# thimabru1010/ResUnet-a_mltsk_keras

Measured on AMD Instinct MI355X. Metric: training patches/sec (256×256, 6-ch, bs=8/GPU) at 1/2/4/8 MI355X, higher is better.
Workload: dtype bf16; 1 GPU; cfg3: ResUnet-a d6 multitask (seg+bound+dist+color) Tanimoto-dual, 256x256x6, 6 classes, Adam, full train step (fwd+loss+bwd+allreduce+update); global_batch=8, per_gpu_batch=8, parallelism=dp1

## Files before the change

include/rua_hip.h:

```cpp
#ifndef RUA_HIP_H
#define RUA_HIP_H
#include <stdint.h>
#ifdef __cplusplus
extern "C" {
#endif

#define RUA_F32 0
#define RUA_BF16 1
#define RUA_MAX_SEG 6
#define RUA_MAX_BRANCH 4
#define RUA_MAX_WGRAD_BATCH 32
#define RUA_MAX_WGRAD_GROUP 8

#define RUA_OK 0
#define RUA_ERR_ARG (-1)
#define RUA_ERR_LAUNCH (-2)

int rua_version(void);
const char* rua_last_error(void);
int rua_device_info(int* cu_count, int* lds_bytes, char* arch, int arch_len);

typedef struct rua_conv_seg {
  const void* x;
  const void* w;
  int32_t C, Hs, Ws;
  int32_t up_shift;
  int32_t dil;
  int32_t taps;
} rua_conv_seg;

typedef struct rua_bn_fold {
  const double* stats;
  int32_t replicas, pad;
  double count, bessel_n;
  float eps, momentum;
  const float* gamma; const float* beta;
  float* moving_mean; float* moving_var;
  float* scale; float* shift; float* mean; float* rstd;
} rua_bn_fold;

typedef struct rua_conv_desc {
  rua_conv_seg seg[RUA_MAX_SEG];
  int32_t nseg;
  int32_t N, H, W, Cout;
  int32_t stride;
  int32_t dtype;
  const float* bias;
  const void* aux;
  int32_t aux_mode;
  const float* mscale;
  const float* mshift;
  int32_t out_relu;
  int32_t accumulate;
  void* y;
  int32_t out_stride, OH, OW;
  double* stats;
  int32_t stats_mode;
  void* workspace;
  int64_t workspace_bytes;
  int32_t stats_replicas;
  const float* bias_more[3];
  const float* in_scale;
  const float* in_shift;
  int32_t in_relu;
  int32_t pad_fold;
  const struct rua_bn_fold* in_fold;
} rua_conv_desc;
int rua_conv_fwd(const rua_conv_desc* d, void* stream);
int rua_conv_fwd_group(const rua_conv_desc* d, int n, void* stream);
int rua_conv_group_last_grids(void);
int rua_conv_group_band_ok(const rua_conv_desc* d, int n);
int rua_conv_group_last_band(void);
int rua_conv_group_last_chain(void);
int rua_conv_fwd_sum(const rua_conv_desc* d, int n, void* stream);
int rua_conv_sum_last_kernel(void);
int rua_conv_sum_kernel(const rua_conv_desc* d, int n);
int rua_conv_smem_bytes(const rua_conv_desc* d);
int64_t rua_conv_workspace_bytes(const rua_conv_desc* d);
void* rua_prof_event_create(void);
int rua_prof_event_record(void* ev, void* hip_stream);
int rua_prof_event_elapsed_us(void* start, void* stop, double* us);
void rua_prof_event_destroy(void* ev);
void rua_profile_mid_event(void* hip_event);
int rua_profile_mid_event_fired(void);
int rua_conv_last_ksplit(void);
int rua_conv_tile_bn(const rua_conv_desc* d);
int rua_conv_kernel_id(const rua_conv_desc* d);
int rua_conv_fused_input_ok(const rua_conv_desc* d);
int rua_conv_tile_bm(const rua_conv_desc* d);

typedef struct rua_wgrad_desc {
  const void* a;  int32_t C, Hs, Ws;
  const void* dy; int32_t Cout, H, W;
  int32_t N, stride, dil, taps, dtype;
  float* dw;
  void* workspace;
  int64_t workspace_bytes;
  const float* in_scale;
  const float* in_shift;
  int32_t in_relu;
  int32_t defer;
  int32_t group_members;
  int32_t batch;
  const int32_t* overwrite_dev;
} rua_wgrad_desc;
typedef struct rua_wgrad_pending {
  int32_t kind;
  int32_t parts;
  int64_t n;
  const float* partials;
  float* dw;
  int32_t CC;
  int32_t blocks;
  int32_t block_begin, pad;
  const int32_t* overwrite_dev;
} rua_wgrad_pending;
int rua_wgrad_plan(const rua_wgrad_desc* d, rua_wgrad_pending* out);
int rua_wgrad_reduce_batch(const rua_wgrad_pending* items_dev, int n_items, int total_blocks, void* stream);
int rua_conv_wgrad(const rua_wgrad_desc* d, void* stream);
int rua_conv_wgrad_group(const rua_wgrad_desc* d, int n, void* stream);
int rua_wgrad_group_last_grids(void);
int rua_wgrad_group_plan(const rua_wgrad_desc* d, int n, rua_wgrad_pending* out);
int64_t rua_wgrad_workspace_bytes(const rua_wgrad_desc* d);
int rua_wgrad_kind(const rua_wgrad_desc* d);
int rua_wgrad_img_kind(const rua_wgrad_desc* d);

typedef struct rua_wprep_item { int64_t src_off, dst_off; int32_t taps, Cout, C, pad; } rua_wprep_item;
int rua_weight_prep(const float* master, void* w_fwd, void* w_dgrad, const rua_wprep_item* items_dev,
                    int n_items, int max_elems, int dtype, void* stream);
int rua_weight_prep_dgrad(const void* w_fwd, void* w_dgrad, const rua_wprep_item* items_dev, int n_items, int max_elems, const int32_t* blockmap_dev,
                          int n_blocks, int dtype, void* stream);
int rua_wprep_blocks(int taps, int Cout, int C);

int rua_stem_fwd(const float* x, const float* w, const float* b, void* y, int64_t M, int Cin, int Cout, int dtype, void* stream);
int rua_stem_fwd_stats(const float* x, const float* w, const float* b, void* y, int64_t M, int Cin, int Cout, int dtype, double* stats, int replicas, void* stream);
int rua_stem_bwd(const float* x, const void* dy, float* dw, float* db, int64_t M, int Cin, int Cout, int dtype, void* stream);
int rua_stem_fwd_pack(const float* x, const float* w, const float* b, void* y, int64_t M, int Cin, int Cout, int dtype, double* stats, int replicas,
                      void* xpack, void* stream);
int rua_stem_bwd_fold(float* tmp, float* dw, float* db, int Cin, int Cout, void* stream);
int rua_head_fwd(const void* x, const float* w, const float* b, float* z, float* p, int64_t M, int Cin, int Cout, int act, int dtype, void* stream);
int rua_head_fwd_loss(const void* x, const float* w, const float* b, float* z, float* p, const float* y, double* tanimoto_sums,
                      double* metrics, int B, int64_t HW, int Cin, int Cout, int act, int dtype, void* stream);
int rua_head_fwd_loss_rep(const void* x, const float* w, const float* b, float* z, float* p, const float* y, double* tanimoto_sums,
                          int sums_replicas, double* metrics, int B, int64_t HW, int Cin, int Cout, int act, int dtype, void* stream);
int rua_head_bwd(const void* x, const float* dz, const float* w, void* dx, int accumulate_dx, float* dw, float* db,
                 float* scratch, int64_t scratch_bytes, int64_t M, int Cin, int Cout, int dtype, int mask_dx, void* stream);
int rua_head_bwd_sums(const void* x, const float* dz, const float* w, void* dx, int accumulate_dx, float* dw, float* db, float* dxsum,
                      float* scratch, int64_t scratch_bytes, int64_t M, int Cin, int Cout, int dtype, int mask_dx, void* stream);

int rua_col_stats(const void* x, int64_t M, int C, double* stats, int replicas, int dtype, void* stream);
int rua_stats_replicas(int64_t blocks);
int rua_col_stats2(const void* g, const void* x, const float* mscale, const float* mshift, int masked,
                   int64_t M, int C, double* stats, int replicas, int dtype, void* stream);
int rua_bn_finalize(const double* stats, int replicas, double count, double bessel_n, const float* gamma, const float* beta,
                    float* moving_mean, float* moving_var, float momentum, float eps, int training,
                    float* scale, float* shift, float* mean, float* rstd, int C, void* stream);
int rua_stats_to_f32(const double* stats, int replicas, int C, float* const* dst, int n, void* stream);
int rua_bn_apply(const void* x, int nb, const float* const* scale, const float* const* shift, int relu,
                 void* const* out, int64_t M, int C, int dtype, void* stream);
int rua_bn_bwd_finalize(const double* stats2, int replicas, double count, const float* gamma, const float* mean, const float* rstd,
                        float* dgamma, float* dbeta, float* coefA, float* coefB, float* coefC, int C, void* stream);
int rua_bn_bwd_apply(int nb, const void* const* g, const float* const* coefA, const float* const* coefB,
                     const float* const* coefC, const float* const* mscale, const float* const* mshift, int masked,
                     const void* x, const void* dskip, void* dx, int accumulate, int64_t M, int C, int dtype, void* stream);

typedef struct rua_bn_branch {
  const float* gamma; const float* beta; float* moving_mean; float* moving_var;
  float* scale; float* shift; float* mean; float* rstd;
  void* out;
  const double* stats; int32_t replicas, pad;
  double* out_stats;
} rua_bn_branch;
typedef struct rua_bn_fwd_desc {
  const void* x; int64_t M; int32_t C, dtype, nb, relu, training, replicas;
  const double* stats;
  double count, bessel_n; float momentum, eps;
  rua_bn_branch br[RUA_MAX_BRANCH];
} rua_bn_fwd_desc;
int rua_bn_fwd(const rua_bn_fwd_desc* d, void* stream);
int rua_bn_fwd_group(const rua_bn_fwd_desc* d, int n, void* stream);
int rua_bn_fwd_group_last_grids(void);
typedef struct rua_bn_bwd_branch {
  const void* g; const double* stats2; int32_t replicas;
  int32_t stats2_out;
  const float* gamma; const float* mean; const float* rstd; const float* scale; const float* shift;
  float* dgamma; float* dbeta;
} rua_bn_bwd_branch;
typedef struct rua_bn_bwd_desc {
  const void* x; const void* dskip; void* dx; int64_t M; int32_t C, dtype, nb, masked, accumulate, pad; double count;
  rua_bn_bwd_branch br[RUA_MAX_BRANCH];
  double* skip_stats;
  int32_t skip_replicas, pad2;
  double* dx_stats;
  int32_t dx_replicas, pad3;
} rua_bn_bwd_desc;
int rua_bn_bwd(const rua_bn_bwd_desc* d, void* stream);
int rua_bn_bwd_group(const rua_bn_bwd_desc* d, int n, void* stream);
int rua_bn_bwd_group_last_grids(void);

int rua_maxpool_fwd(const void* x, void* y, uint8_t* idx, int N, int H, int W, int C, int k, int dtype, void* stream);
int rua_maxpool_bwd(const void* dy, const uint8_t* idx, void* dx, int accumulate, int N, int H, int W, int C, int k, int dtype, void* stream);
int rua_sumpool(const void* x, void* y, int N, int H, int W, int C, int k, int dtype, void* stream);
int rua_maxpool_derive(const void* y_half, const uint8_t* idx_half, void* y, uint8_t* idx, int N, int H_half, int W_half, int C,
                       int k_half, int dtype, void* stream);
int rua_maxpool_bwd_multi(int n, const void* const* dy, const uint8_t* const* idx, const int* ks, void* dx, int accumulate,
                          int N, int H, int W, int C, int dtype, void* stream);
int rua_sumpool_pyramid(const void* x, void* y2, void* y4, void* y8, int N, int H, int W, int C, int dtype, void* stream);
int rua_upsample_nearest(const void* x, void* y, int N, int H, int W, int C, int k, int dtype, void* stream);

int rua_add_n(int n, const void* const* in, void* out, int accumulate, int64_t elems, int dtype, void* stream);
int rua_relu_mask(void* dy, const void* y, int64_t elems, int dtype, void* stream);
int rua_relu(const void* x, void* y, int64_t elems, int dtype, void* stream);
int rua_cast_f32_to(const float* x, void* y, int64_t elems, int dtype, void* stream);
int rua_cast_to_f32(const void* x, float* y, int64_t elems, int dtype, void* stream);
int rua_fill_zero(void* p, int64_t bytes, void* stream);

#define RUA_LOSS_TANIMOTO 0
#define RUA_LOSS_WCE 1
#define RUA_LOSS_CE_LOGITS 2
#define RUA_LOSS_BCE_LOGITS 3
#define RUA_LOSS_MSE 4
#define RUA_ACT_NONE 0
#define RUA_ACT_SOFTMAX 1
#define RUA_ACT_SIGMOID 2
int rua_tanimoto_sums(const float* p, const float* y, int B, int64_t HW, int C, double* sums, void* stream);
int rua_tanimoto_finalize(const double* sums, int B, int64_t HW, int C, float grad_scale, double* loss_out, float* coef,
                          float* per_sample, void* stream);
#define RUA_MAX_HEADS 8
typedef struct rua_tani_head {
  double* sums; int32_t replicas, B, C; float grad_scale; double* loss_out; float* coef; float* per_sample;
} rua_tani_head;
int rua_tanimoto_finalize_multi(const rua_tani_head* heads, int n, void* stream);
typedef struct rua_dz_head {
  int32_t kind, act; const float* p; const float* y; const float* coef; const float* class_w; float grad_scale; int32_t B; int64_t HW; int32_t C, pad; float* dz;
} rua_dz_head;
int rua_head_dz_multi(const rua_dz_head* heads, int n, void* stream);
int rua_tanimoto_finalize_rep(double* sums, int replicas, int B, int64_t HW, int C, float grad_scale, double* loss_out, float* coef,
                              float* per_sample, void* stream);
int rua_tanimoto_ratio(const double* sums, int B, int C, double* mean_out, float* per_sample, void* stream);
int rua_pixel_loss(int kind, const float* p, const float* z, const float* y, const float* class_w,
                   int64_t M, int C, double* loss_out, float* per_pixel, void* stream);
int rua_head_dz(int kind, int act, const float* p, const float* y, const float* coef, const float* class_w,
                float grad_scale, int B, int64_t HW, int C, float* dz, void* stream);
int rua_seg_metrics(const float* p, const float* y, int64_t M, int C, double* out, void* stream);

int rua_tanimoto_sums_void(const float* p, const float* y, const uint8_t* void_mask, int B, int64_t HW, int C, double* sums, void* stream);
int rua_head_fwd_loss_void(const void* x, const float* w, const float* b, float* z, float* p, const float* y, double* tanimoto_sums,
                           int sums_replicas, double* metrics, int B, int64_t HW, int Cin, int Cout, int act, int dtype,
                           const uint8_t* void_mask, void* stream);
int rua_pixel_loss_void(int kind, const float* p, const float* z, const float* y, const float* class_w, const uint8_t* void_mask,
                        int64_t M, int C, double* loss_out, float* per_pixel, void* stream);
int rua_head_dz_void(int kind, int act, const float* p, const float* y, const float* coef, const float* class_w,
                     float grad_scale, int B, int64_t HW, int C, const uint8_t* void_mask, float* dz, void* stream);
int rua_head_dz_multi_void(const rua_dz_head* heads, int n, const uint8_t* void_mask, void* stream);
int rua_seg_metrics_void(const float* p, const float* y, const uint8_t* void_mask, int64_t M, int C, double* out, void* stream);

int rua_lr_step(double* state, float* lr_out, int adam, double beta1, double beta2, void* stream);
int rua_adam_step(float* theta, float* g, float* m, float* v, int64_t n, float lr_t, const float* lr_t_dev, float beta1, float beta2,
                  float eps, float grad_scale, int zero_grad, void* stream);
int rua_sgd_step(float* theta, float* g, float* vel, int64_t n, float lr, const float* lr_dev, float momentum, float grad_scale,
                 int zero_grad, void* stream);
int rua_adam_step_w(float* theta, float* g, float* m, float* v, int64_t n, float lr_t, const float* lr_t_dev, float beta1, float beta2,
                    float eps, float grad_scale, int zero_grad, void* wcopy_bf16, void* stream);
int rua_sgd_step_w(float* theta, float* g, float* vel, int64_t n, float lr, const float* lr_dev, float momentum, float grad_scale,
                   int zero_grad, void* wcopy_bf16, void* stream);

int64_t rua_targets_scratch_bytes(int N, int num_classes);
int rua_multitask_targets(const uint8_t* img, const uint8_t* cls, int N, int H, int W, int Cin, int num_classes, int norm_type,
                          float* x, float* seg, float* bound, float* dist, float* color, void* scratch, int64_t scratch_bytes, void* stream);
int rua_void_mask(const uint8_t* cls, int N, int H, int W, int num_classes, int margin, uint8_t* mask, void* stream);

int rua_scene_windows(const uint8_t* const* scene_img, const uint8_t* const* scene_cls, const int32_t* scene_h, const int32_t* scene_w,
                      int nscenes, const int32_t* windows, int N, int PH, int PW, int Cin,
                      uint8_t* img_out, uint8_t* cls_out, void* stream);

int rua_scene_windows_affine(const uint8_t* const* scene_img, const uint8_t* const* scene_cls, const int32_t* scene_h, const int32_t* scene_w,
                             int nscenes, const int32_t* windows , int N, int PH, int PW, int Cin,
// ... 36 lines not shown
```

resunet_a_mltsk_keras_amd/_lib.py:

```python
from __future__ import annotations

import ctypes as C
import os

HERE = os.path.dirname(os.path.abspath(__file__))
LIB_PATH = os.environ.get("RUA_LIB_PATH") or os.path.join(HERE, "librua_hip.so")

RUA_F32, RUA_BF16 = 0, 1
RUA_MAX_SEG, RUA_MAX_BRANCH, RUA_MAX_WGRAD_GROUP, RUA_MAX_WGRAD_BATCH = 6, 4, 8, 32
LOSS_TANIMOTO, LOSS_WCE, LOSS_CE_LOGITS, LOSS_BCE_LOGITS, LOSS_MSE = 0, 1, 2, 3, 4
ACT_NONE, ACT_SOFTMAX, ACT_SIGMOID = 0, 1, 2

vp, i32, i64, f32, f64 = C.c_void_p, C.c_int32, C.c_int64, C.c_float, C.c_double


class ConvSeg(C.Structure):
    _fields_ = [("x", vp), ("w", vp), ("C", i32), ("Hs", i32), ("Ws", i32), ("up_shift", i32), ("dil", i32), ("taps", i32)]


class ConvDesc(C.Structure):
    _fields_ = [("seg", ConvSeg * RUA_MAX_SEG), ("nseg", i32), ("N", i32), ("H", i32), ("W", i32), ("Cout", i32),
                ("stride", i32), ("dtype", i32), ("bias", vp), ("aux", vp), ("aux_mode", i32), ("mscale", vp),
                ("mshift", vp), ("out_relu", i32), ("accumulate", i32), ("y", vp), ("out_stride", i32), ("OH", i32),
                ("OW", i32), ("stats", vp), ("stats_mode", i32), ("workspace", vp), ("workspace_bytes", i64), ("stats_replicas", i32),
                ("bias_more", vp * 3), ("in_scale", vp), ("in_shift", vp), ("in_relu", i32), ("pad_fold", i32), ("in_fold", vp)]


class BnFold(C.Structure):
    _fields_ = [("stats", vp), ("replicas", i32), ("pad", i32), ("count", f64), ("bessel_n", f64), ("eps", f32), ("momentum", f32),
                ("gamma", vp), ("beta", vp), ("moving_mean", vp), ("moving_var", vp), ("scale", vp), ("shift", vp), ("mean", vp), ("rstd", vp)]


class WgradDesc(C.Structure):
    _fields_ = [("a", vp), ("C", i32), ("Hs", i32), ("Ws", i32), ("dy", vp), ("Cout", i32), ("H", i32), ("W", i32),
                ("N", i32), ("stride", i32), ("dil", i32), ("taps", i32), ("dtype", i32), ("dw", vp), ("workspace", vp), ("workspace_bytes", i64),
                ("in_scale", vp), ("in_shift", vp), ("in_relu", i32), ("defer", i32), ("group_members", i32), ("batch", i32), ("overwrite_dev", vp)]


class WgradPending(C.Structure):
    _fields_ = [("kind", i32), ("parts", i32), ("n", i64), ("partials", vp), ("dw", vp), ("CC", i32), ("blocks", i32),
                ("block_begin", i32), ("pad", i32), ("overwrite_dev", vp)]


class TaniHead(C.Structure):
    _fields_ = [("sums", vp), ("replicas", i32), ("B", i32), ("C", i32), ("grad_scale", f32), ("loss_out", vp), ("coef", vp), ("per_sample", vp)]


class DzHead(C.Structure):
    _fields_ = [("kind", i32), ("act", i32), ("p", vp), ("y", vp), ("coef", vp), ("class_w", vp), ("grad_scale", f32), ("B", i32), ("HW", i64),
                ("C", i32), ("pad", i32), ("dz", vp)]


class BnBranch(C.Structure):
    _fields_ = [("gamma", vp), ("beta", vp), ("moving_mean", vp), ("moving_var", vp), ("scale", vp), ("shift", vp),
                ("mean", vp), ("rstd", vp), ("out", vp), ("stats", vp), ("replicas", i32), ("pad", i32), ("out_stats", vp)]


class BnFwdDesc(C.Structure):
    _fields_ = [("x", vp), ("M", i64), ("C", i32), ("dtype", i32), ("nb", i32), ("relu", i32), ("training", i32), ("replicas", i32),
                ("stats", vp), ("count", f64), ("bessel_n", f64), ("momentum", f32), ("eps", f32), ("br", BnBranch * RUA_MAX_BRANCH)]


class BnBwdBranch(C.Structure):
    _fields_ = [("g", vp), ("stats2", vp), ("replicas", i32), ("stats2_out", i32), ("gamma", vp), ("mean", vp), ("rstd", vp),
                ("scale", vp), ("shift", vp), ("dgamma", vp), ("dbeta", vp)]


class BnBwdDesc(C.Structure):
    _fields_ = [("x", vp), ("dskip", vp), ("dx", vp), ("M", i64), ("C", i32), ("dtype", i32), ("nb", i32), ("masked", i32),
                ("accumulate", i32), ("pad", i32), ("count", f64), ("br", BnBwdBranch * RUA_MAX_BRANCH),
                ("skip_stats", vp), ("skip_replicas", i32), ("pad2", i32), ("dx_stats", vp), ("dx_replicas", i32), ("pad3", i32)]


class WprepItem(C.Structure):
    _fields_ = [("src_off", i64), ("dst_off", i64), ("taps", i32), ("Cout", i32), ("C", i32), ("pad", i32)]


PP = C.POINTER(vp)

_SIGS = {
    "rua_version": ([], i32),
    "rua_device_info": ([C.POINTER(i32), C.POINTER(i32), C.c_char_p, i32], i32),
    "rua_conv_fwd": ([C.POINTER(ConvDesc), vp], i32),
    "rua_conv_fwd_group": ([C.POINTER(ConvDesc), i32, vp], i32),
    "rua_conv_smem_bytes": ([C.POINTER(ConvDesc)], i32),
    "rua_conv_tile_bn": ([C.POINTER(ConvDesc)], i32),
    "rua_conv_tile_bm": ([C.POINTER(ConvDesc)], i32),
    "rua_conv_kernel_id": ([C.POINTER(ConvDesc)], i32),
    "rua_conv_fused_input_ok": ([C.POINTER(ConvDesc)], i32),
    "rua_conv_last_ksplit": ([], i32),
    "rua_conv_group_last_grids": ([], i32),
    "rua_conv_group_band_ok": ([C.POINTER(ConvDesc), i32], i32),
    "rua_conv_group_last_band": ([], i32),
    "rua_conv_group_last_chain": ([], i32),
    "rua_conv_fwd_sum": ([C.POINTER(ConvDesc), i32, vp], i32),
    "rua_conv_sum_last_kernel": ([], i32),
    "rua_conv_sum_kernel": ([C.POINTER(ConvDesc), i32], i32),
    "rua_conv_wgrad_group": ([C.POINTER(WgradDesc), i32, vp], i32),
    "rua_wgrad_group_last_grids": ([], i32),
    "rua_wgrad_group_plan": ([C.POINTER(WgradDesc), i32, C.POINTER(WgradPending)], i32),
    "rua_profile_mid_event": ([vp], None),
    "rua_profile_mid_event_fired": ([], i32),
    "rua_prof_event_create": ([], vp),
    "rua_prof_event_record": ([vp, vp], i32),
    "rua_prof_event_elapsed_us": ([vp, vp, C.POINTER(f64)], i32),
    "rua_prof_event_destroy": ([vp], None),
    "rua_graph_kernel_nodes": ([vp, C.POINTER(i32), C.POINTER(i32)], i32),
    "rua_conv_workspace_bytes": ([C.POINTER(ConvDesc)], i64),
    "rua_conv_wgrad": ([C.POINTER(WgradDesc), vp], i32),
    "rua_wgrad_workspace_bytes": ([C.POINTER(WgradDesc)], i64),
    "rua_wgrad_kind": ([C.POINTER(WgradDesc)], i32),
    "rua_wgrad_img_kind": ([C.POINTER(WgradDesc)], i32),
    "rua_wgrad_plan": ([C.POINTER(WgradDesc), C.POINTER(WgradPending)], i32),
    "rua_wgrad_reduce_batch": ([vp, i32, i32, vp], i32),
    "rua_weight_prep": ([vp, vp, vp, vp, i32, i32, i32, vp], i32),
    "rua_weight_prep_dgrad": ([vp, vp, vp, i32, i32, vp, i32, i32, vp], i32),
    "rua_wprep_blocks": ([i32, i32, i32], i32),
    "rua_stem_fwd": ([vp, vp, vp, vp, i64, i32, i32, i32, vp], i32),
    "rua_stem_fwd_stats": ([vp, vp, vp, vp, i64, i32, i32, i32, vp, i32, vp], i32),
    "rua_stem_bwd": ([vp, vp, vp, vp, i64, i32, i32, i32, vp], i32),
    "rua_stem_fwd_pack": ([vp, vp, vp, vp, i64, i32, i32, i32, vp, i32, vp, vp], i32),
    "rua_stem_bwd_fold": ([vp, vp, vp, i32, i32, vp], i32),
    "rua_head_fwd": ([vp, vp, vp, vp, vp, i64, i32, i32, i32, i32, vp], i32),
    "rua_head_fwd_loss": ([vp, vp, vp, vp, vp, vp, vp, vp, i32, i64, i32, i32, i32, i32, vp], i32),
    "rua_head_fwd_loss_rep": ([vp, vp, vp, vp, vp, vp, vp, i32, vp, i32, i64, i32, i32, i32, i32, vp], i32),
    "rua_head_bwd": ([vp, vp, vp, vp, i32, vp, vp, vp, i64, i64, i32, i32, i32, i32, vp], i32),
    "rua_head_bwd_sums": ([vp, vp, vp, vp, i32, vp, vp, vp, vp, i64, i64, i32, i32, i32, i32, vp], i32),
    "rua_col_stats": ([vp, i64, i32, vp, i32, i32, vp], i32),
    "rua_col_stats2": ([vp, vp, vp, vp, i32, i64, i32, vp, i32, i32, vp], i32),
    "rua_stats_replicas": ([i64], i32),
    "rua_bn_finalize": ([vp, i32, f64, f64, vp, vp, vp, vp, f32, f32, i32, vp, vp, vp, vp, i32, vp], i32),
    "rua_bn_apply": ([vp, i32, PP, PP, i32, PP, i64, i32, i32, vp], i32),
    "rua_bn_bwd_finalize": ([vp, i32, f64, vp, vp, vp, vp, vp, vp, vp, vp, i32, vp], i32),
    "rua_bn_bwd_apply": ([i32, PP, PP, PP, PP, PP, PP, i32, vp, vp, vp, i32, i64, i32, i32, vp], i32),
    "rua_stats_to_f32": ([vp, i32, i32, PP, i32, vp], i32),
    "rua_bn_fwd": ([C.POINTER(BnFwdDesc), vp], i32),
    "rua_bn_fwd_group": ([C.POINTER(BnFwdDesc), i32, vp], i32),
    "rua_bn_fwd_group_last_grids": ([], i32),
    "rua_bn_bwd": ([C.POINTER(BnBwdDesc), vp], i32),
    "rua_bn_bwd_group": ([C.POINTER(BnBwdDesc), i32, vp], i32),
    "rua_bn_bwd_group_last_grids": ([], i32),
    "rua_maxpool_fwd": ([vp, vp, vp, i32, i32, i32, i32, i32, i32, vp], i32),
    "rua_maxpool_bwd": ([vp, vp, vp, i32, i32, i32, i32, i32, i32, i32, vp], i32),
    "rua_sumpool": ([vp, vp, i32, i32, i32, i32, i32, i32, vp], i32),
    "rua_maxpool_derive": ([vp, vp, vp, vp, i32, i32, i32, i32, i32, i32, vp], i32),
    "rua_maxpool_bwd_multi": ([i32, vp, vp, vp, vp, i32, i32, i32, i32, i32, i32, vp], i32),
    "rua_sumpool_pyramid": ([vp, vp, vp, vp, i32, i32, i32, i32, i32, vp], i32),
    "rua_upsample_nearest": ([vp, vp, i32, i32, i32, i32, i32, i32, vp], i32),
    "rua_add_n": ([i32, PP, vp, i32, i64, i32, vp], i32),
    "rua_relu_mask": ([vp, vp, i64, i32, vp], i32),
    "rua_relu": ([vp, vp, i64, i32, vp], i32),
    "rua_cast_f32_to": ([vp, vp, i64, i32, vp], i32),
    "rua_cast_to_f32": ([vp, vp, i64, i32, vp], i32),
    "rua_fill_zero": ([vp, i64, vp], i32),
    "rua_tanimoto_sums": ([vp, vp, i32, i64, i32, vp, vp], i32),
    "rua_tanimoto_finalize": ([vp, i32, i64, i32, f32, vp, vp, vp, vp], i32),
    "rua_tanimoto_finalize_rep": ([vp, i32, i32, i64, i32, f32, vp, vp, vp, vp], i32),
    "rua_tanimoto_finalize_multi": ([vp, i32, vp], i32),
    "rua_head_dz_multi": ([vp, i32, vp], i32),
    "rua_tanimoto_ratio": ([vp, i32, i32, vp, vp, vp], i32),
    "rua_pixel_loss": ([i32, vp, vp, vp, vp, i64, i32, vp, vp, vp], i32),
    "rua_head_dz": ([i32, i32, vp, vp, vp, vp, f32, i32, i64, i32, vp, vp], i32),
    "rua_seg_metrics": ([vp, vp, i64, i32, vp, vp], i32),
    "rua_lr_step": ([vp, vp, i32, f64, f64, vp], i32),
    "rua_adam_step": ([vp, vp, vp, vp, i64, f32, vp, f32, f32, f32, f32, i32, vp], i32),
    "rua_sgd_step": ([vp, vp, vp, i64, f32, vp, f32, f32, i32, vp], i32),
    "rua_adam_step_w": ([vp, vp, vp, vp, i64, f32, vp, f32, f32, f32, f32, i32, vp, vp], i32),
    "rua_sgd_step_w": ([vp, vp, vp, i64, f32, vp, f32, f32, i32, vp, vp], i32),
    "rua_tanimoto_sums_void": ([vp, vp, vp, i32, i64, i32, vp, vp], i32),
    "rua_head_fwd_loss_void": ([vp, vp, vp, vp, vp, vp, vp, i32, vp, i32, i64, i32, i32, i32, i32, vp, vp], i32),
    "rua_pixel_loss_void": ([i32, vp, vp, vp, vp, vp, i64, i32, vp, vp, vp], i32),
    "rua_head_dz_void": ([i32, i32, vp, vp, vp, vp, f32, i32, i64, i32, vp, vp, vp], i32),
    "rua_head_dz_multi_void": ([vp, i32, vp, vp], i32),
    "rua_seg_metrics_void": ([vp, vp, vp, i64, i32, vp, vp], i32),
    "rua_void_mask": ([vp, i32, i32, i32, i32, i32, vp, vp], i32),
    "rua_targets_scratch_bytes": ([i32, i32], i64),
    "rua_multitask_targets": ([vp, vp, i32, i32, i32, i32, i32, i32, vp, vp, vp, vp, vp, vp, i64, vp], i32),
    "rua_scene_windows": ([vp, vp, vp, vp, i32, vp, i32, i32, i32, i32, vp, vp, vp], i32),
    "rua_scene_windows_affine": ([vp, vp, vp, vp, i32, vp, i32, i32, i32, i32, vp, vp, vp], i32),
    "rua_scene_stitch": ([vp, i32, i32, i32, i32, vp, vp, vp, vp, vp, vp, i32, vp, vp], i32),
    "rua_scene_stitch_views": ([vp, i32, i32, i32, i32, i32, vp, vp, vp, vp, vp, vp, i32, vp, vp], i32),
    "rua_scene_stitch_maps": ([vp, i32, i32, i32, i32, i32, vp, vp, vp, vp, vp, i32, i32, vp], i32),
    "rua_scene_class_counts": ([vp, vp, vp, i32, vp, i32, i32, i32, i32, vp, vp], i32),
    "rua_scene_erode": ([vp, vp, vp, i32, i32, vp, vp, i32, vp, vp], i32),
    "rua_scene_boundary": ([vp, vp, vp, vp, i32, i32, i32, vp, vp, vp, vp], i32),
    "rua_set_tuning": ([C.c_char_p, i64], i32),
    "rua_get_tuning": ([C.c_char_p, C.POINTER(i64)], i32),
    "rua_tuning_key": ([i32], C.c_char_p),
}

EXPORTED_SYMBOLS = sorted(list(_SIGS) + ["rua_last_error"])


class RuaError(RuntimeError):
    pass


class _Lib:
    def __init__(self):
        if not os.path.exists(LIB_PATH):
            raise RuaError(
                f"{LIB_PATH} is missing: the HIP extension has not been built. Run "
                "`python -m resunet_a_mltsk_keras_amd.build` (needs hipcc). There is no CPU fallback.")
        self.dll = C.CDLL(LIB_PATH)
        self.dll.rua_last_error.restype = C.c_char_p
        self.dll.rua_last_error.argtypes = []
        for name, (args, res) in _SIGS.items():
            fn = getattr(self.dll, name)
            fn.argtypes = args
            fn.restype = res
            setattr(self, "_" + name, fn)

        i = 0
        while True:
            key = self.dll.rua_tuning_key(i) if hasattr(self.dll, "rua_tuning_key") else None
            if not key:
                break
            v = os.environ.get("RUA_TUNE_" + key.decode().upper())
            if v is not None:
                self.check(self.dll.rua_set_tuning(key, int(v)), "rua_set_tuning")
            i += 1

    def set_tuning(self, **kv):
        for k, v in kv.items():
            self.check(self.dll.rua_set_tuning(k.encode(), int(v)), "rua_set_tuning")

    def get_tuning(self, key: str) -> int:
        v = i64()
        self.check(self.dll.rua_get_tuning(key.encode(), C.byref(v)), "rua_get_tuning")
        return int(v.value)

    def raw(self, name):
        return getattr(self, "_" + name)

    def check(self, rc, name):
        if rc != 0:
            raise RuaError(f"{name} failed ({rc}): {self.dll.rua_last_error().decode()}")

    def call(self, name, *args):
        self.check(getattr(self, "_" + name)(*args), name)


_lib = None


def lib() -> _Lib:
    global _lib
    if _lib is None:
        _lib = _Lib()
    return _lib


def ptr_array(ptrs):
    arr = (vp * len(ptrs))(*[vp(p) for p in ptrs])
    return arr
```

resunet_a_mltsk_keras_amd/csrc/conv_img2.hip:

```cpp
#include "common.h"

struct Img2K {
  const unsigned char* x; const unsigned char* w; float* ws;
  int C, Cout, H, M, ngrp, nco, ksplit, cpb;
  unsigned xbytes, wbytes;
};
template <int V> struct Img2IC { static constexpr int value = V; };

template <int W>
__device__ __forceinline__ void conv_img2_body(const Img2K& q) {
  constexpr int NW = 8, HW = W * W, PXB = 256, NPX = 256;
  constexpr int XB = NPX * PXB, ZOFF = XB, SWO = XB + 256;
  constexpr int KS = 8, TAPB = 64 * PXB, WBUF = 3 * TAPB, WPW = (WBUF / 1024) / NW, XPW = (XB / 1024) / NW;
  extern __shared__ __attribute__((aligned(16))) unsigned char smem[];
  const int tid = threadIdx.x, lane = tid & 63;
  const int wv = __builtin_amdgcn_readfirstlane(tid >> 6);
  const int pl = lane & 31, kh = lane >> 5;
  const int pg = wv >> 1, coh = wv & 1;
  const int nwg = (int)gridDim.x, bid = blockIdx.x;
  const int xcd = bid & 7, q8 = nwg >> 3, r8 = nwg & 7;
  const int job = (xcd < r8 ? xcd * (q8 + 1) : r8 * (q8 + 1) + (xcd - r8) * q8) + (bid >> 3);
  const int cs = job % q.nco, t1 = job / q.nco;
  const int ks = t1 % q.ksplit, grp = t1 / q.ksplit;
  const int m0 = grp * NPX, co0 = cs * 64, ch0 = ks * q.cpb;
  const int C = q.C;
  if (tid < 16) *reinterpret_cast<uint4*>(smem + ZOFF + tid * 16) = make_uint4(0, 0, 0, 0);

  const int qd0 = wv * 4 + (lane >> 4);
  const int psrc = (lane & 15) ^ (qd0 & 15);
  const __amdgpu_buffer_rsrc_t rx = make_rsrc(q.x, q.xbytes), rw = make_rsrc(q.w, q.wbytes);
  const unsigned xsrc = (unsigned)(((m0 + qd0) * C + psrc * 8) * 2);
  auto issue_x = [&](int ch) {
#pragma unroll
    for (int k = 0; k < XPW; ++k)
      __builtin_amdgcn_raw_ptr_buffer_load_lds(rx, (lds_void_p)(smem + (k * NW + wv) * 1024), 16, xsrc + (unsigned)((k * 32 * C + ch * 128) * 2), 0, 0, 0);
  };
  const int wrow0 = 4 * (wv & 3) + (lane >> 4);
  const unsigned wsrc = (unsigned)(((co0 + wrow0) * C + (((lane & 15) ^ wrow0) * 8)) * 2);
  auto issue_w1 = [&](int ch, int ty, int i, bool ok) {
    const int idx = i * NW + wv;
    const unsigned off = ok ? wsrc + (unsigned)((((ty * 3 + (idx >> 4)) * q.Cout + 16 * ((idx & 15) >> 2)) * C + ch * 128) * 2) : 0x80000000u;
    __builtin_amdgcn_raw_ptr_buffer_load_lds(rw, (lds_void_p)(smem + SWO + idx * 1024), 16, off, 0, 0, 0);
  };
  auto frag = [&](unsigned e, int k) { return *reinterpret_cast<const bf16x8*>(smem + (e ^ (unsigned)(k << 5))); };
  auto eaddr = [&](unsigned base, int row) {
    const int sw = row & 15;
    return base + (unsigned)(row * PXB + ((sw >> 1) << 5) + (((kh ^ sw) & 1) << 4));
  };
  const unsigned ew0 = eaddr((unsigned)SWO, coh * 32 + pl);
  auto wfrag = [&](int tx, int k) { return frag(ew0 + (unsigned)(tx * TAPB), k); };
  int qy[2], qx[2], qq[2];
#pragma unroll
  for (int t = 0; t < 2; ++t) { qq[t] = pg * 64 + t * 32 + pl; qy[t] = (qq[t] % HW) / W; qx[t] = qq[t] % W; }

  f32x16 acc[2];
#pragma unroll
  for (int t = 0; t < 2; ++t)
#pragma unroll
    for (int k = 0; k < 16; ++k) acc[t][k] = 0.f;

  issue_x(ch0);
#pragma unroll
  for (int i = 0; i < WPW; ++i) issue_w1(ch0, 0, i, true);
  asm volatile("s_waitcnt vmcnt(0)" ::: "memory");
  __syncthreads();
  bf16x8 wf[3][KS];
#pragma unroll
  for (int tx = 0; tx < 3; ++tx)
#pragma unroll
    for (int k = 0; k < KS; ++k) wf[tx][k] = wfrag(tx, k);
  asm volatile("s_waitcnt lgkmcnt(0)" ::: "memory");

  const int nph = 3 * q.cpb;
  for (int ph = 0; ph < nph; ++ph) {
    const int chl = ph / 3, ty = ph - 3 * chl;
    const int nch = (ph + 1) / 3, nty = (ph + 1) - 3 * nch;
    const bool nok = ph + 1 < nph;
    unsigned eoff[3][2];
#pragma unroll
    for (int tx = 0; tx < 3; ++tx)
#pragma unroll
      for (int t = 0; t < 2; ++t) {
        const int yy = qy[t] + ty - 1, xx = qx[t] + tx - 1;
        const bool in = (unsigned)yy < (unsigned)W && (unsigned)xx < (unsigned)W;
        eoff[tx][t] = in ? eaddr(0u, qq[t] + (ty - 1) * W + (tx - 1)) : (unsigned)ZOFF + (unsigned)(kh << 4);
      }
    auto stage = [&](auto spc) {
      constexpr int sp = decltype(spc)::value;
      __builtin_amdgcn_s_barrier();
      constexpr int NI = 3 * KS, PF = 4, NDMA = sp == 0 ? WPW : 0, D0 = 1, DSTEP = 3;
      bf16x8 fr[8];
#pragma unroll
      for (int i = 0; i < PF; ++i) fr[i] = frag(eoff[i / KS][sp], i % KS);
#pragma unroll
      for (int i = 0; i < NI; ++i) {
        const int tx = i / KS, k = i % KS;
        if (i + PF < NI) fr[(i + PF) & 7] = frag(eoff[(i + PF) / KS][sp], (i + PF) % KS);
        acc[sp] = __builtin_amdgcn_mfma_f32_32x32x16_bf16(wf[tx][k], fr[i & 7], acc[sp], 0, 0, 0);
        if constexpr (sp == 1) wf[tx][k] = wfrag(tx, k);
        if (NDMA > 0 && i >= D0 && (i - D0) % DSTEP == 0 && (i - D0) / DSTEP < NDMA) issue_w1(nch + ch0, nty, (i - D0) / DSTEP, nok);
      }
      __builtin_amdgcn_sched_group_barrier(0x100, PF, 0);
#pragma unroll
      for (int i = 0; i < NI; ++i) {
        __builtin_amdgcn_sched_group_barrier(0x008, 1, 0);
        if (i + PF < NI) __builtin_amdgcn_sched_group_barrier(0x100, 1 + sp, 0);
        else if (sp == 1) __builtin_amdgcn_sched_group_barrier(0x100, 1, 0);
        if (NDMA > 0 && i >= D0 && (i - D0) % DSTEP == 0 && (i - D0) / DSTEP < NDMA) __builtin_amdgcn_sched_group_barrier(0x010, 1, 0);
      }
      asm volatile("s_waitcnt vmcnt(0)\n\ts_waitcnt lgkmcnt(0)" ::: "memory");
    };
    stage(Img2IC<0>{});
    stage(Img2IC<1>{});
    if (ty == 2 && chl + 1 < q.cpb) {
      __builtin_amdgcn_s_barrier();
      issue_x(ch0 + chl + 1);
      asm volatile("s_waitcnt vmcnt(0)" ::: "memory");
    }
  }
  float* slab = q.ws + ((size_t)ks * q.M + m0) * q.Cout + co0 + coh * 32 + 8 * kh;
#pragma unroll
  for (int t = 0; t < 2; ++t) {
    float* row = slab + (size_t)qq[t] * q.Cout;
#pragma unroll
    for (int g = 0; g < 2; ++g) {
      f32x4 lo, hi;
#pragma unroll
      for (int j = 0; j < 4; ++j) {
        float a = acc[t][(2 * g) * 4 + j], b2 = acc[t][(2 * g + 1) * 4 + j];
        if (g == 0 && j == 0) asm volatile("s_nop 7\n\ts_nop 7\n\ts_nop 7\n\tv_permlane32_swap_b32 %0, %1" : "+v"(a), "+v"(b2));
        else asm volatile("s_nop 1\n\tv_permlane32_swap_b32 %0, %1" : "+v"(a), "+v"(b2));
        lo[j] = a; hi[j] = b2;
      }
      *reinterpret_cast<f32x4*>(row + 16 * g) = lo;
      *reinterpret_cast<f32x4*>(row + 16 * g + 4) = hi;
    }
  }
}
template <int W> __global__ __launch_bounds__(512) void conv_img2(const Img2K q) { conv_img2_body<W>(q); }

int rua_pick_img2(const rua_conv_desc* d) {
  if (!g_tune.conv_img2 || g_conv_group || d->dtype != RUA_BF16 || d->nseg != 1 || d->in_scale || d->in_fold) return 0;
  const rua_conv_seg& g = d->seg[0];
  if (g.taps != 9 || g.dil != 1 || d->stride != 1 || d->out_stride != 1 || g.up_shift != 0 || g.Hs != d->H || g.Ws != d->W || d->H != d->W || (d->W != 8 && d->W != 16) ||
      d->OH != d->H || d->OW != d->W) return 0;
  if (g.C % 128 || d->Cout % 64) return 0;
  const long long M = (long long)d->N * d->H * d->W;
  if (M % 256 || M * d->Cout * 4 >= (1ll << 31) || M * g.C * 2 >= 0x7FFFFF00ll || 9ll * d->Cout * g.C * 2 >= 0x7FFFFF00ll) return 0;
  const int nchunk = g.C / 128, groups = (int)(M / 256) * (d->Cout / 64);
  const size_t ws_usable = d->workspace_bytes > 4096 ? (size_t)d->workspace_bytes - 4096 : 0;
  const long long slabs = d->workspace ? (long long)(ws_usable / ((size_t)M * d->Cout * sizeof(float))) : 0;
  int ks = (rua_cu_count() + groups - 1) / groups;
  if (ks > nchunk) ks = nchunk;
  if (ks > slabs) ks = (int)slabs;
  while (ks > 1 && nchunk % ks) --ks;
  if (ks < 2) return 0;
  return ks;
}

int rua_launch_conv_img2(ConvK& k, const rua_conv_desc* d, int KS, hipStream_t st) {
  const rua_conv_seg& g = d->seg[0];
  Img2K q;
  q.x = (const unsigned char*)g.x; q.w = (const unsigned char*)g.w; q.ws = (float*)d->workspace;
  q.C = g.C; q.Cout = d->Cout; q.H = d->H; q.M = (int)k.M; q.ngrp = (int)(k.M / 256); q.nco = d->Cout / 64; q.ksplit = KS; q.cpb = (g.C / 128) / KS;
  q.xbytes = (unsigned)((size_t)k.M * g.C * 2); q.wbytes = (unsigned)((size_t)9 * d->Cout * g.C * 2);
  k.nbn = (d->Cout + 63) / 64; k.nbm = (int)(k.M / 256); k.ksplit = KS; k.stages_per_split = 0; k.ws = (float*)d->workspace; k.cnt = nullptr;
  const unsigned grid = (unsigned)(q.ngrp * q.nco * KS);
  constexpr int smem = 256 * 256 + 256 + 3 * 64 * 256;
  static RuaPerDevFlag attr;
  if (!attr.get()) {
    (void)hipFuncSetAttribute(reinterpret_cast<const void*>(&conv_img2<8>), hipFuncAttributeMaxDynamicSharedMemorySize, smem);
    (void)hipFuncSetAttribute(reinterpret_cast<const void*>(&conv_img2<16>), hipFuncAttributeMaxDynamicSharedMemorySize, smem);
    attr.get() = true;
  }
  if (d->W == 8) hipLaunchKernelGGL((conv_img2<8>), dim3(grid), dim3(512), smem, st, q);
  else hipLaunchKernelGGL((conv_img2<16>), dim3(grid), dim3(512), smem, st, q);
  RUA_LAUNCH_CHECK("conv_img2");
  return rua_splitk_finish_bf16(k, st);
}
```

resunet_a_mltsk_keras_amd/csrc/conv_mfma.hip:

```cpp
#include "common.h"


template <typename T> __device__ __forceinline__ void load8(const unsigned char* base, size_t elem_off, float* f) {
  if constexpr (sizeof(T) == 2) {
    ET<T>::unpack(ldg16(base + elem_off * 2), f);
  } else {
    ET<T>::unpack(ldg16(base + elem_off * 4), f);
    ET<T>::unpack(ldg16(base + elem_off * 4 + 16), f + 4);
  }
}
template <typename T> __device__ __forceinline__ void store8(unsigned char* base, size_t elem_off, const float* f) {
  if constexpr (sizeof(T) == 2) {
    stg16(base + elem_off * 2, ET<T>::pack(f));
  } else {
    stg16(base + elem_off * 4, ET<T>::pack(f));
    stg16(base + elem_off * 4 + 16, ET<T>::pack(f + 4));
  }
}

template <typename T, int BM, int BN> __host__ __device__ constexpr int conv_smem_base() {
  constexpr int ROWB = (sizeof(T) == 2) ? 80 : 132;
  constexpr int a = 2 * (BM + BN) * ROWB;
  constexpr int b = BM * (BN + 4) * 4 + 4 * (BN / 8) * 16 * 4;
  return ((a > b ? a : b) + 15) / 16 * 16;
// ... 1662 lines not shown
  const int lr = lane & 31, lh = lane >> 5;
  const int bn_i = blockIdx.x % p.nbn, bm_i = blockIdx.x / p.nbn;
  const long long m0 = (long long)bm_i * BM;
  const int n0 = bn_i * BN;
  const long long m = m0 + lr;
  const bool av = m < p.M;
  const int mm = av ? (int)m : 0, HW = p.H * p.W;
  const int n = mm / HW, rem = mm - n * HW, h = rem / p.W, w = rem - h * p.W;
  const int ah = h * p.stride, aw = w * p.stride;
  int total = 0;
  for (int s_ = 0; s_ < p.nseg; ++s_) total += p.seg[s_].C >> 4;
  const int q = (total + 3) >> 2;
  int ks = wid * q, ke = ks + q < total ? ks + q : total;
  int seg = 0, kk = ks;
  while (seg + 1 < p.nseg && kk >= (p.seg[seg].C >> 4)) { kk -= p.seg[seg].C >> 4; ++seg; }
  f32x16 acc[BNT];
#pragma unroll
  for (int t = 0; t < BNT; ++t)
#pragma unroll
    for (int i = 0; i < 16; ++i) acc[t][i] = 0.f;
  __amdgpu_buffer_rsrc_t rx = make_rsrc(p.seg[0].x, p.seg[0].xbytes), rw = make_rsrc(p.seg[0].w, p.seg[0].wbytes);
  unsigned abase = OOB, bbase[BNT];
  int nk = 1;
  auto enter = [&]() {
    const SegK sg = p.seg[seg];
    rx = make_rsrc(sg.x, sg.xbytes); rw = make_rsrc(sg.w, sg.wbytes);
    nk = sg.C >> 4;
    abase = av ? (unsigned)((((n * sg.Hs + (ah >> sg.up)) * sg.Ws + (aw >> sg.up)) * sg.C + lh * 8) * 2) : OOB;
#pragma unroll
    for (int t = 0; t < BNT; ++t) bbase[t] = (n0 + t * 32 + lr) < p.Cout ? (unsigned)(((n0 + t * 32 + lr) * sg.C + lh * 8) * 2) : OOB;
  };
  if (ks < ke) enter();
  while (ks < ke) {
    int nstep = ke - ks;
    if (nstep > CH) nstep = CH;
    if (nstep > nk - kk) nstep = nk - kk;
    uint4 a[CH], b[BNT][CH];
#pragma unroll
    for (int j = 0; j < CH; ++j)
      if (j < nstep) {
        a[j] = bufload16(rx, abase + (unsigned)((kk + j) * 32));
#pragma unroll
        for (int t = 0; t < BNT; ++t) b[t][j] = bufload16(rw, bbase[t] + (unsigned)((kk + j) * 32));
      }
#pragma unroll
    for (int j = 0; j < CH; ++j)
      if (j < nstep) {
#pragma unroll
        for (int t = 0; t < BNT; ++t)
          acc[t] = __builtin_amdgcn_mfma_f32_32x32x16_bf16(__builtin_bit_cast(bf16x8, a[j]), __builtin_bit_cast(bf16x8, b[t][j]), acc[t], 0, 0, 0);
      }
    ks += nstep; kk += nstep;
    if (kk == nk && ks < ke) { ++seg; kk = 0; enter(); }
  }
  float* mine = part + wid * BM * CSTR;
#pragma unroll
  for (int t = 0; t < BNT; ++t)
#pragma unroll
    for (int i = 0; i < 16; ++i) mine[((i & 3) + 8 * (i >> 2) + 4 * lh) * CSTR + t * 32 + lr] = acc[t][i];
  __syncthreads();
  for (int e = tid; e < BM * BN; e += 256) {
    const int r = e / BN, c = e - r * BN, o = r * CSTR + c;
    part[o] = ((part[o] + part[BM * CSTR + o]) + part[2 * BM * CSTR + o]) + part[3 * BM * CSTR + o];
  }
  __syncthreads();
  conv_epilogue<T, BM, BN>(p, m0, n0, bm_i, part, CSTR, sred);
}
template <int BNT> __global__ __launch_bounds__(256) void conv_small(const ConvK p) { conv_small_body<BNT>(p); }
template <int BNT> __global__ __launch_bounds__(256) void conv_small_g(const ConvKG g) {
  const ConvK& p = g.k[blockIdx.y];
  if ((int)blockIdx.x >= p.nbm * p.nbn) return;
  conv_small_body<BNT>(p);
}

static bool pick_small(const rua_conv_desc* d) {
  if (!g_tune.conv_small || d->dtype != RUA_BF16 || d->in_scale || d->in_fold) return false;
  const long long M = (long long)d->N * d->H * d->W;
  if (M > g_tune.conv_small || d->Cout < 32) return false;
  for (int s_ = 0; s_ < d->nseg; ++s_)
    if (d->seg[s_].taps != 1 || d->seg[s_].C % 16 != 0) return false;
  return true;
}
static int launch_conv_small(ConvK& k, hipStream_t st) {
  k.nbm = (int)((k.M + 31) / 32); k.nbn = (k.Cout + 63) / 64;
  k.ksplit = 1; k.stages_per_split = 0; k.ws = nullptr; k.cnt = nullptr;
  constexpr int smem = (4 * 32 * 68 + 4 * 8 * 16) * 4;
  if (g_conv_group && (g_tune.conv_group & 16)) {
    if (!g_conv_group->add(7, (unsigned)(k.nbm * k.nbn), smem, k)) { rua_set_error("rua_conv_fwd_group: more than %d captured members", RUA_MAX_BRANCH); return RUA_ERR_ARG; }
    return RUA_OK;
  }
  hipLaunchKernelGGL((conv_small<2>), dim3(k.nbm * k.nbn), dim3(256), smem, st, k);
  RUA_LAUNCH_CHECK("conv_small");
  return RUA_OK;
}

static thread_local int g_last_ksplit = 1;
extern "C" int rua_conv_last_ksplit(void) { return g_last_ksplit; }

extern "C" int rua_conv_fwd(const rua_conv_desc* d, void* stream) {
  RUA_CHECK_ARG(d && d->nseg >= 1 && d->nseg <= RUA_MAX_SEG, "rua_conv_fwd: nseg out of range");
  RUA_CHECK_ARG(d->dtype == RUA_F32 || d->dtype == RUA_BF16, "rua_conv_fwd: bad dtype");
  const int vec = d->dtype == RUA_BF16 ? 8 : 4;
  RUA_CHECK_ARG(d->Cout > 0 && d->Cout % 8 == 0, "rua_conv_fwd: Cout=%d must be a multiple of 8", d->Cout);
  RUA_CHECK_ARG(d->N > 0 && d->H > 0 && d->W > 0 && d->stride >= 1, "rua_conv_fwd: bad output grid");
  RUA_CHECK_ARG(d->y != nullptr, "rua_conv_fwd: null output");
  RUA_CHECK_ARG(d->out_stride >= 1 && d->OH >= (d->H - 1) * d->out_stride + 1 && d->OW >= (d->W - 1) * d->out_stride + 1,
                "rua_conv_fwd: output tensor smaller than the strided grid");
  RUA_CHECK_ARG((long long)d->N * d->H * d->W < (1ll << 31), "rua_conv_fwd: too many pixels");
  RUA_CHECK_ARG(d->aux_mode == 0 || d->aux != nullptr, "rua_conv_fwd: aux_mode without aux");
  RUA_CHECK_ARG(d->stats_mode == 0 || d->stats != nullptr, "rua_conv_fwd: stats_mode without stats");
  RUA_CHECK_ARG(d->stats_mode != 2 || d->aux != nullptr, "rua_conv_fwd: stats_mode 2 needs aux");
  ConvK k;
  k.nseg = d->nseg;
  int units = 0;
  for (int s = 0; s < d->nseg; ++s) {
    const rua_conv_seg& g = d->seg[s];
    RUA_CHECK_ARG(g.x && g.w, "rua_conv_fwd: null segment pointer");
    RUA_CHECK_ARG(g.C > 0 && g.C % vec == 0, "rua_conv_fwd: segment C=%d not a multiple of %d", g.C, vec);
    RUA_CHECK_ARG(g.taps == 1 || g.taps == 9, "rua_conv_fwd: taps must be 1 or 9");
    RUA_CHECK_ARG(g.up_shift >= 0 && g.up_shift <= 4 && g.dil >= 1, "rua_conv_fwd: bad up_shift/dil");
    RUA_CHECK_ARG((long long)(d->H - 1) * d->stride < ((long long)g.Hs << g.up_shift) &&
                  (long long)(d->W - 1) * d->stride < ((long long)g.Ws << g.up_shift),
                  "rua_conv_fwd: segment %d source %dx%d (up %d) too small for output %dx%d stride %d", s, g.Hs, g.Ws, g.up_shift, d->H, d->W, d->stride);
    RUA_CHECK_ARG((long long)d->N * g.Hs * g.Ws * g.C * 4 < (1ll << 31), "rua_conv_fwd: source tensor must stay below 2 GiB (32-bit offsets)");
    RUA_CHECK_ARG(g.up_shift == 0 || g.taps == 1, "rua_conv_fwd: nearest-upsampled sources are 1x1 only");
    RUA_CHECK_ARG((long long)g.taps * d->Cout * g.C * 4 < (1ll << 31), "rua_conv_fwd: weight block too large");
    SegK& o = k.seg[s];
    o.x = (const unsigned char*)g.x; o.w = (const unsigned char*)g.w;
    o.C = g.C; o.Hs = g.Hs; o.Ws = g.Ws; o.up = g.up_shift; o.dil = g.dil; o.taps = g.taps;
    o.nchunk = (g.C + 31) / 32; o.ubegin = units;
    o.xbytes = (unsigned)((size_t)d->N * g.Hs * g.Ws * g.C * (d->dtype == RUA_BF16 ? 2 : 4));
    o.wbytes = (unsigned)((size_t)g.taps * d->Cout * g.C * (d->dtype == RUA_BF16 ? 2 : 4));
    units += g.taps * o.nchunk;
  }
  k.nunits = units;
  RUA_CHECK_ARG(units <= RUA_MAX_UNITS, "rua_conv_fwd: K = %d units of 32 channels exceeds the unit-table capacity %d", units, RUA_MAX_UNITS);
  k.N = d->N; k.H = d->H; k.W = d->W; k.Cout = d->Cout; k.stride = d->stride;
  k.M = (long long)d->N * d->H * d->W;
  k.bias = d->bias; k.aux = (const unsigned char*)d->aux; k.aux_mode = d->aux_mode;
  for (int q = 0; q < 3; ++q) k.bias_more[q] = d->bias ? d->bias_more[q] : nullptr;
  k.mscale = d->mscale; k.mshift = d->mshift; k.out_relu = d->out_relu; k.accumulate = d->accumulate;
  k.y = (unsigned char*)d->y; k.out_stride = d->out_stride; k.OH = d->OH; k.OW = d->OW;
  k.stats = d->stats; k.stats_mode = d->stats_mode;
  k.stats_R = d->stats_replicas < 1 ? 1 : d->stats_replicas;
  RUA_CHECK_ARG((k.stats_R & (k.stats_R - 1)) == 0, "rua_conv_fwd: stats_replicas must be a power of two");
  k.in_scale = d->in_scale; k.in_shift = d->in_shift; k.in_relu = d->in_relu;
  k.epi_fast = g_tune.epi_fast;
  hipStream_t st = (hipStream_t)stream;
  if (rua_pick_strip(d)) {
    k.nbn = 1; k.nbm = 1; k.ksplit = 1; k.stages_per_split = 0; k.ws = nullptr; k.cnt = nullptr;
    g_last_ksplit = 1;
    return rua_launch_conv_strip(k, d, st);
  }
  RUA_CHECK_ARG(d->in_scale == nullptr && d->in_fold == nullptr, "rua_conv_fwd: in_scale / in_shift / in_fold (normalise on load) is not available for "
                                        "this shape: ask rua_conv_fused_input_ok() first");
  if (pick_halo(d)) {
    k.nbn = 1; k.nbm = 1; k.ksplit = 1; k.stages_per_split = 0; k.ws = nullptr; k.cnt = nullptr;
    g_last_ksplit = 1;
    return launch_conv_halo(k, d->seg[0].dil, st);
  }
  if (pick_pw(d)) {
    k.nbn = 1; k.nbm = 1; k.ksplit = 1; k.stages_per_split = 0; k.ws = nullptr; k.cnt = nullptr;
    g_last_ksplit = 1;
    const int ks = pw_steps(d);
    return ks <= 2 ? launch_conv_pw<2>(k, d, st) : ks <= 4 ? launch_conv_pw<4>(k, d, st) : launch_conv_pw<6>(k, d, st);
  }
  if (pick_small(d)) {
    g_last_ksplit = 1;
    return launch_conv_small(k, st);
  }
  if (const int img2_ks = rua_pick_img2(d)) {
    g_last_ksplit = img2_ks;
    return rua_launch_conv_img2(k, d, img2_ks, st);
  }
  if (!g_conv_group && rua_band128_sum_ok(d)) {
    g_last_ksplit = 1;
    return rua_launch_band128_sum(d, st);
  }
  if (const int img_ks = pick_img(d)) {
    g_last_ksplit = img_ks;
    return launch_conv_img(k, d, img_ks, st);
  }
  if (pick_dmap(d)) {
    const int target = g_tune.dmap_target > 0 ? g_tune.dmap_target : rua_cu_count();
    k.nbn = (d->Cout + 127) / 128;
    k.nbm = (int)((k.M + 127) / 128);
    const int nstages = units / 2;
    const long long tiles = (long long)k.nbm * k.nbn;
    int want = 1;
    const int fused = g_tune.dmap_fused_finish;
    const size_t ws_usable = d->workspace_bytes > 4096 ? (size_t)d->workspace_bytes - 4096 : 0;
    const long long slabs = d->workspace ? (long long)(ws_usable / ((size_t)k.M * d->Cout * sizeof(float))) : 0;
    k.cnt = (fused && d->workspace && tiles <= 1024) ? reinterpret_cast<int*>((char*)d->workspace + ws_usable) : nullptr;
    if (slabs >= 2 && tiles < target) {
      want = (int)((target + tiles - 1) / tiles);
      if (want > nstages / 4) want = nstages / 4;
      if (want > 32) want = 32;
      if (want > slabs) want = (int)slabs;
      if (want < 1) want = 1;
      if (tiles * 2 >= target && nstages <= 40) want = 1;
    }
    k.ws = (float*)d->workspace;
    k.stages_per_split = (nstages + want - 1) / want;
    k.ksplit = (nstages + k.stages_per_split - 1) / k.stages_per_split;
    g_last_ksplit = k.ksplit;
    const int rowb = g_tune.dmap_rowb == 128 ? 128 : 64;
    const int bm64 = g_tune.dmap_bm64;
    if (bm64 && k.ksplit == 1 && tiles < target && tiles * 2 >= target) {
      k.nbm = (int)((k.M + 63) / 64);
      return launch_conv_dmap<64, 128, 64>(k, st);
    }
    return rowb == 128 ? launch_conv_dmap<128, 128, 128>(k, st) : launch_conv_dmap<128, 128, 64>(k, st);
  }
  const int bn = pick_bn(d, k.M);
  int bm = pick_bm(d, k.M, bn);
  k.nbn = (d->Cout + bn - 1) / bn;
  int nbm = (int)((k.M + bm - 1) / bm);
  k.nbm = nbm;
  const int nstages = (units + 1) / 2;
  k.ws = (float*)d->workspace;
  k.cnt = nullptr;
  k.ksplit = (d->workspace && bm == 128) ? pick_ksplit((long long)nbm * k.nbn, nstages, k.M, d->Cout,
                                                       d->workspace_bytes > 4096 ? (size_t)d->workspace_bytes - 4096 : 0) : 1;
  k.stages_per_split = (nstages + k.ksplit - 1) / k.ksplit;
  k.ksplit = (nstages + k.stages_per_split - 1) / k.stages_per_split;
  g_last_ksplit = k.ksplit;
  if (pick_dma(d, bn)) return dispatch_conv_dma(k, bm, bn, nbm, st);
  if (d->dtype == RUA_BF16) return dispatch_conv<bf16_t>(k, bm, bn, nbm, st);
  return dispatch_conv<float>(k, bm, bn, nbm, st);
}

thread_local ConvGroupCapture* g_conv_group = nullptr;
static thread_local int g_group_last_grids = 0;
static thread_local int g_group_last_band = 0;
extern "C" int rua_conv_group_last_grids(void) { return g_group_last_grids; }
static thread_local int g_group_last_chain = 0;
extern "C" int rua_conv_group_last_chain(void) { return g_group_last_chain; }
extern "C" int rua_conv_group_last_band(void) { return g_group_last_band; }
extern "C" int rua_conv_group_band_ok(const rua_conv_desc* d, int n) { return (d && (rua_band64m_ok(d, n) || rua_band128m_ok(d, n))) ? 1 : 0; }

template <typename KG, typename F1, typename FG>
static int issue_group(const ConvGroupCapture& c, const int* idx, int m, F1 single, FG grouped, int smem_attr, hipStream_t st, const char* what) {
  if (m == 1) {
    hipLaunchKernelGGL(single, dim3(c.grid[idx[0]]), dim3(256), c.smem[idx[0]], st, c.k[idx[0]]);
  } else {
    static RuaPerDevFlag attr[8];
    const int slot = c.kind[idx[0]];
    if (!attr[slot].get()) { (void)hipFuncSetAttribute(reinterpret_cast<const void*>(grouped), hipFuncAttributeMaxDynamicSharedMemorySize, smem_attr); attr[slot].get() = true; }
    KG g;
    for (int i = 0; i < m; ++i) g.k[i] = c.k[idx[i]];
    hipLaunchKernelGGL(grouped, dim3(c.grid[idx[0]], m), dim3(256), c.smem[idx[0]], st, g);
  }
  RUA_LAUNCH_CHECK(what);
  return RUA_OK;
}

static bool chain_ok(const ConvGroupCapture& c, const int* idx, int m) {
  const ConvK& a = c.k[idx[0]];
  for (int i = 0; i < m; ++i) {
    const ConvK& k = c.k[idx[i]];
    if (k.ksplit != 1 || k.M != a.M || k.Cout != a.Cout || k.nbm != a.nbm || k.nbn != a.nbn || k.H != a.H || k.W != a.W || k.stride != a.stride) return false;
  }
  return true;
}
template <typename FC>
static int issue_chain(const ConvGroupCapture& c, const int* idx, int m, FC kern, int smem, int slot, hipStream_t st) {
  static RuaPerDevFlag attr[2];
  if (!attr[slot].get()) { (void)hipFuncSetAttribute(reinterpret_cast<const void*>(kern), hipFuncAttributeMaxDynamicSharedMemorySize, smem); attr[slot].get() = true; }
  ConvKG g;
  for (int i = 0; i < m; ++i) g.k[i] = c.k[idx[i]];
  hipLaunchKernelGGL(kern, dim3(c.grid[idx[0]]), dim3(256), smem, st, g, m);
  RUA_LAUNCH_CHECK("conv_dmap_chain");
  return RUA_OK;
}

extern "C" int rua_conv_fwd_group(const rua_conv_desc* d, int n, void* stream) {
  RUA_CHECK_ARG(d && n >= 1 && n <= RUA_MAX_BRANCH, "rua_conv_fwd_group: 1..%d members", RUA_MAX_BRANCH);
  hipStream_t st = (hipStream_t)stream;
  g_group_last_grids = n;
  g_group_last_band = 0;
  g_group_last_chain = 0;
  if (n >= 2 && rua_band128m_ok(d, n)) {
    const int rc = rua_launch_band128m(d, n, st);
    if (rc == RUA_OK) { g_group_last_grids = 1; g_group_last_band = 2; }
    return rc;
  }
  if (rua_band64m_ok(d, n)) {
    const int rc = rua_launch_band64m(d, n, st);
    if (rc == RUA_OK) { g_group_last_grids = 1; g_group_last_band = 1; }
    return rc;
  }
  if (n == 1 || !g_tune.conv_group) {
    for (int i = 0; i < n; ++i) { const int rc = rua_conv_fwd(d + i, stream); if (rc != RUA_OK) return rc; }
    return RUA_OK;
  }
  ConvGroupCapture cap;
  cap.n = 0;
  cap.members = n;
  PwGroupCapture pwc;
  pwc.n = 0;
  rua_strip_group_reset();
  g_conv_group = &cap;
  g_pw_group = (g_tune.conv_group & 32) ? &pwc : nullptr;
  int rc = RUA_OK;
  for (int i = 0; i < n && rc == RUA_OK; ++i) rc = rua_conv_fwd(d + i, stream);
  g_conv_group = nullptr;
  g_pw_group = nullptr;
  if (rc != RUA_OK) { rua_strip_group_reset(); return rc; }
  int grids = n - cap.n - pwc.n - rua_strip_group_pending();
  for (int dense = 0; dense < 2; ++dense) {
    PwKG<2> g; int m = 0; unsigned gx = 0;
    for (int i = 0; i < pwc.n; ++i) if ((int)pwc.dense[i] == dense) { g.k[m++] = pwc.k[i]; if ((unsigned)pwc.k[i].nblk > gx) gx = (unsigned)pwc.k[i].nblk; }
    if (m == 0) continue;
    for (int i = m; i < RUA_MAX_BRANCH; ++i) g.k[i] = g.k[0];
    if (m == 1) { if (dense) hipLaunchKernelGGL((conv_pw<2, true>), dim3(gx), dim3(256), 0, st, g.k[0]); else hipLaunchKernelGGL((conv_pw<2, false>), dim3(gx), dim3(256), 0, st, g.k[0]); }
    else if (dense) hipLaunchKernelGGL((conv_pw_g<2, true>), dim3(gx, m), dim3(256), 0, st, g);
    else hipLaunchKernelGGL((conv_pw_g<2, false>), dim3(gx, m), dim3(256), 0, st, g);
    RUA_LAUNCH_CHECK("conv_pw (group)");
    ++grids;
  }
  rc = rua_strip_group_flush(st, &grids);
  if (rc != RUA_OK) return rc;
  bool done[RUA_MAX_BRANCH] = {false};
  for (int i = 0; i < cap.n; ++i) {
    if (done[i]) continue;
    int idx[RUA_MAX_BRANCH], m = 0;
    if (cap.kind[i] == 7) {
      unsigned gmax = 0;
      for (int j = i; j < cap.n; ++j)
        if (!done[j] && cap.kind[j] == 7) { idx[m++] = j; done[j] = true; if (cap.grid[j] > gmax) gmax = cap.grid[j]; }
      if (m == 1) hipLaunchKernelGGL((conv_small<2>), dim3(cap.grid[idx[0]]), dim3(256), cap.smem[idx[0]], st, cap.k[idx[0]]);
      else { ConvKG g; for (int q = 0; q < m; ++q) g.k[q] = cap.k[idx[q]]; hipLaunchKernelGGL((conv_small_g<2>), dim3(gmax, m), dim3(256), cap.smem[idx[0]], st, g); }
      RUA_LAUNCH_CHECK("conv_small (group)");
      ++grids;
      continue;
    }
    for (int j = i; j < cap.n; ++j)
      if (!done[j] && cap.kind[j] == cap.kind[i] && cap.grid[j] == cap.grid[i] && cap.smem[j] == cap.smem[i]) { idx[m++] = j; done[j] = true; }
    const bool chain = m >= 2 && (cap.kind[i] == 1 || cap.kind[i] == 2) && (g_tune.dmap_chain & cap.kind[i]) && chain_ok(cap, idx, m);
    if (chain) g_group_last_chain = m;
    if (chain && cap.kind[i] == 1) rc = issue_chain(cap, idx, m, conv_dmap_chain<128, 128, 64>, conv_dmap_chain_smem<128, 128>(), 0, st);
    else if (chain) rc = issue_chain(cap, idx, m, conv_dmap_chain<64, 128, 64>, conv_dmap_chain_smem<64, 128>(), 1, st);
    else if (cap.kind[i] == 1) rc = issue_group<ConvKG>(cap, idx, m, conv_dmap<128, 128, 64>, conv_dmap_g<128, 128, 64>, conv_dmap_smem<128, 128>(), st, "conv_dmap (group)");
    else if (cap.kind[i] == 6) rc = issue_group<ConvKG>(cap, idx, m, conv_dmap_s<128, 128, 64>, conv_dmap_gs<128, 128, 64>, conv_dmap_smem<128, 128, 4>(), st, "conv_dmap_s (group)");
    else if (cap.kind[i] == 2) rc = issue_group<ConvKG>(cap, idx, m, conv_dmap<64, 128, 64>, conv_dmap_g<64, 128, 64>, conv_dmap_smem<64, 128>(), st, "conv_dmap (group)");
    else rc = issue_group<ConvKG>(cap, idx, m, conv_igemm<bf16_t, 256, 64>, conv_igemm_g<bf16_t, 256, 64>, conv_smem<bf16_t, 256, 64>(), st, "conv_igemm (group)");
    if (rc != RUA_OK) return rc;
    ++grids;
  }
  g_group_last_grids = grids;
  return RUA_OK;
}

extern "C" int64_t rua_conv_workspace_bytes(const rua_conv_desc* d) {
  if (!d) return 0;
  return (int64_t)d->N * d->H * d->W * d->Cout * (int64_t)sizeof(float);
}

extern "C" int rua_conv_tile_bn(const rua_conv_desc* d) {
  if (!d) return RUA_ERR_ARG;
  if (pick_dmap(d)) return 128;
  return pick_bn(d, (long long)d->N * d->H * d->W);
}
extern "C" int rua_conv_fused_input_ok(const rua_conv_desc* d) { return (d && rua_pick_strip(d)) ? 1 : 0; }

extern "C" int rua_conv_kernel_id(const rua_conv_desc* d) {
  if (!d) return RUA_ERR_ARG;
  if (rua_pick_strip(d)) return 5;
  if (pick_halo(d)) return 3;
  if (pick_pw(d)) return 4;
  if (pick_small(d)) return 6;
  if (rua_pick_img2(d)) return 8;
  if (!g_conv_group && rua_band128_sum_ok(d)) return 9;
  if (pick_img(d)) return 7;
  if (pick_dmap(d)) return 2;
  return pick_dma(d, pick_bn(d, (long long)d->N * d->H * d->W)) ? 1 : 0;
}
extern "C" int rua_conv_tile_bm(const rua_conv_desc* d) {
  if (!d) return RUA_ERR_ARG;
  const long long M = (long long)d->N * d->H * d->W;
  if (pick_dmap(d)) {
    const int target = g_tune.dmap_target > 0 ? g_tune.dmap_target : rua_cu_count();
    const int bm64 = g_tune.dmap_bm64;
    const long long tiles = ((M + 127) / 128) * ((d->Cout + 127) / 128);
    int units = 0;
    for (int i = 0; i < d->nseg; ++i) units += d->seg[i].taps * (d->seg[i].C / 32);
    const bool split = d->workspace && d->workspace_bytes > 4096 &&
                       (size_t)(d->workspace_bytes - 4096) / ((size_t)M * d->Cout * sizeof(float)) >= 2 && units / 2 > 40;
    return (bm64 && !split && tiles < target && tiles * 2 >= target) ? 64 : 128;
  }
  return pick_bm(d, M, pick_bn(d, M));
}
```

resunet_a_mltsk_keras_amd/csrc/conv_wgrad.hip:

```cpp
#include "common.h"

static thread_local bool g_wgrad_dry = false;
static thread_local rua_wgrad_pending* g_wgrad_pending = nullptr;
static inline void note_pending(int kind, int parts, long long n, const float* partials, float* dw, int CC, int blocks) {
  if (!g_wgrad_pending) return;
  g_wgrad_pending->kind = kind; g_wgrad_pending->parts = parts; g_wgrad_pending->n = n; g_wgrad_pending->partials = partials;
  g_wgrad_pending->dw = dw; g_wgrad_pending->CC = CC; g_wgrad_pending->blocks = blocks;
}

struct WgK {
  const unsigned char* a; const unsigned char* dy; float* dw;
  int C, Hs, Ws, Cout, H, W, N, stride, dil, taps;
  long long M; int pix_per_block, ntc, nti, ksplit;
  int wshift, hshift;
  float* slabs;
  const int* overwrite;
};

template <typename T>
__device__ __forceinline__ void wgrad_kernel_body(const WgK& p, int b) {
  constexpr int VEC = ET<T>::VEC, ES = sizeof(T);
  constexpr int TP = 64;
  constexpr int PPR = 64 / VEC;
  constexpr int ROWB = (ES == 2) ? 192 : 260;
// ... 836 lines not shown
  }
  auto xslot = [&](int rho) { return (unsigned)(((rho + 1 + R) % R) * SLOT); };
  auto dslot = [&](int j) { return (unsigned)(((j + RD) % RD) * DSLOT); };
  auto issue = [&](int xr, int dr) {
    const bool xok_ = SX ? (xr <= sn && G.is_row(cxi)) : xrow_ok(xr);
    const bool dok_ = SX ? (dr >= 0 && dr < sn && G.is_row(cdi)) : (dr >= 0 && dr < nit);
    const unsigned xbase = xok_ ? (unsigned)(SX ? G.grow(cxi) : n_ * H + r_ + (i0 + xr) * d) * rowbytes : OOB;
    const unsigned dbase = dok_ ? (unsigned)(SX ? G.grow(cdi) : n_ * H + r_ + (i0 + dr) * d) * rowbytes : OOB;
    if constexpr (SX) { G.adv(cxi); if (dr >= 0) G.adv(cdi); }
    const unsigned xs = xslot(xr), ds = dslot(dr);
#pragma unroll
    for (int k = 0; k < KDMA; ++k) {
      const int pi = k * NW + wv;
      if (pi < NPS) __builtin_amdgcn_raw_ptr_buffer_load_lds(rx, (lds_void_p)(sX + xs + pi * 1024), 16, (xbase + (unsigned)(pi * 1024)) + srel, 0, 0, 0);
      else if (pi < 2 * NPS) __builtin_amdgcn_raw_ptr_buffer_load_lds(rd, (lds_void_p)(sDy + ds + (pi - NPS) * 1024), 16, (dbase + (unsigned)((pi - NPS) * 1024)) + srel, 0, 0, 0);
      else { const unsigned z = 0u, off = OOB; asm volatile("buffer_store_dword %0, %1, %2, 0 offen" :: "v"(z), "v"(off), "s"(rd) : "memory"); }
    }
  };
  auto transform = [&](int rho) {
    if constexpr (BN) {
      const bool tok_ = SX ? (rho <= sn && G.is_row(ctr)) : xrow_ok(rho);
      if constexpr (SX) G.adv(ctr);
      const unsigned ca = (tab_a + (tok_ ? 0u : 128u * 4u)) + (unsigned)(gchunk * 32);
      const unsigned xs = sx_a + xslot(rho) + lrel;
#pragma unroll
      for (int k = 0; k < KDMA; ++k) {
        const int pi = k * NW + wv;
        if (pi < NPS) {
          u32x4_t rw; f32x4 sa, sb, ha, hb;
          const unsigned a = xs + (unsigned)(pi * 1024);
          asm volatile("ds_read_b128 %0, %5\n\tds_read_b128 %1, %6\n\tds_read_b128 %2, %6 offset:16\n\tds_read_b128 %3, %6 offset:256\n\tds_read_b128 %4, %6 offset:272\n\t"
                       "s_waitcnt lgkmcnt(0)" : "=&v"(rw), "=&v"(sa), "=&v"(sb), "=&v"(ha), "=&v"(hb) : "v"(a), "v"(ca) : "memory");
          float f[8];
          ET<bf16_t>::unpack(make_uint4(rw[0], rw[1], rw[2], rw[3]), f);
#pragma unroll
          for (int j = 0; j < 4; ++j) { f[j] = fmaf(sa[j], f[j], ha[j]); f[4 + j] = fmaf(sb[j], f[4 + j], hb[j]); }
          typedef __attribute__((ext_vector_type(2))) short s16x2;
          typedef __attribute__((ext_vector_type(2))) float f32x2_t;
          typedef __attribute__((ext_vector_type(2))) __bf16 bf16x2_t;
          const s16x2 z = {0, 0};
#pragma unroll
          for (int j = 0; j < 4; ++j) {
            const f32x2_t p2 = {f[2 * j], f[2 * j + 1]};
            const bf16x2_t b2 = __builtin_convertvector(p2, bf16x2_t);
            rw[j] = __builtin_bit_cast(unsigned, __builtin_elementwise_max(__builtin_bit_cast(s16x2, b2), z));
          }
          asm volatile("ds_write_b128 %0, %1" :: "v"(a), "v"(rw) : "memory");
        }
      }
    }
  };

  f32x16 acc[6];
#pragma unroll
  for (int j = 0; j < 6; ++j)
#pragma unroll
    for (int i = 0; i < 16; ++i) acc[j][i] = 0.f;

  struct Frags { s16x4 d0[2], d1[2], x0[3], x1[3]; };
  auto read_frags = [&](unsigned da, unsigned xa, int ks, Frags& f) {
    const unsigned dk0 = da + (unsigned)(dyo0 + ks * 16 * PXB), dk1 = dk0 ^ 64u;
    const unsigned xk0 = (unsigned)((int)xa + xo0 + ks * 16 * PXB), xk1 = (unsigned)((int)xa + xo1 + ks * 16 * PXB), xk2 = (unsigned)((int)xa + xo2 + ks * 16 * PXB);
    asm volatile("ds_read_b64_tr_b16 %0, %10\n\tds_read_b64_tr_b16 %1, %10 offset:512\n\t"
                 "ds_read_b64_tr_b16 %2, %11\n\tds_read_b64_tr_b16 %3, %11 offset:512\n\t"
                 "ds_read_b64_tr_b16 %4, %12\n\tds_read_b64_tr_b16 %5, %12 offset:512\n\t"
                 "ds_read_b64_tr_b16 %6, %13\n\tds_read_b64_tr_b16 %7, %13 offset:512\n\t"
                 "ds_read_b64_tr_b16 %8, %14\n\tds_read_b64_tr_b16 %9, %14 offset:512"
                 : "=&v"(f.d0[0]), "=&v"(f.d1[0]), "=&v"(f.d0[1]), "=&v"(f.d1[1]), "=&v"(f.x0[0]), "=&v"(f.x1[0]), "=&v"(f.x0[1]), "=&v"(f.x1[1]), "=&v"(f.x0[2]), "=&v"(f.x1[2])
                 : "v"(dk0), "v"(dk1), "v"(xk0), "v"(xk1), "v"(xk2) : "memory");
  };
  auto wait_frags = [&](Frags& f, int pending) {
    if (pending) asm volatile("s_waitcnt lgkmcnt(10)" : "+v"(f.d0[0]), "+v"(f.d1[0]), "+v"(f.d0[1]), "+v"(f.d1[1]), "+v"(f.x0[0]), "+v"(f.x1[0]), "+v"(f.x0[1]), "+v"(f.x1[1]), "+v"(f.x0[2]), "+v"(f.x1[2]) :: "memory");
    else asm volatile("s_waitcnt lgkmcnt(0)" : "+v"(f.d0[0]), "+v"(f.d1[0]), "+v"(f.d0[1]), "+v"(f.d1[1]), "+v"(f.x0[0]), "+v"(f.x1[0]), "+v"(f.x0[1]), "+v"(f.x1[1]), "+v"(f.x0[2]), "+v"(f.x1[2]) :: "memory");
  };
  typedef __attribute__((ext_vector_type(8))) short s16x8;
  auto mfma6 = [&](const Frags& f) {
#pragma unroll
    for (int h = 0; h < 2; ++h) {
      const s16x8 fd = {f.d0[h][0], f.d0[h][1], f.d0[h][2], f.d0[h][3], f.d1[h][0], f.d1[h][1], f.d1[h][2], f.d1[h][3]};
#pragma unroll
      for (int j = 0; j < 3; ++j) {
        const s16x8 fx = {f.x0[j][0], f.x0[j][1], f.x0[j][2], f.x0[j][3], f.x1[j][0], f.x1[j][1], f.x1[j][2], f.x1[j][3]};
        acc[h * 3 + j] = __builtin_amdgcn_mfma_f32_32x32x16_bf16(__builtin_bit_cast(bf16x8, fd), __builtin_bit_cast(bf16x8, fx), acc[h * 3 + j], 0, 0, 0);
      }
    }
  };

  const int njb_ = SX ? 1 : p.jpw;
  for (int jb = 0; jb < njb_; ++jb) {
    if constexpr (SX) nit = sn; else enter_job((int)blockIdx.x + jb * p.gx);
    asm volatile("s_waitcnt vmcnt(0)\n\ts_waitcnt lgkmcnt(0)" ::: "memory");
    __builtin_amdgcn_s_barrier();
    issue(-1, -1); issue(0, 0); issue(1, 1); issue(2, -1);
    asm volatile("s_waitcnt vmcnt(0)" ::: "memory");
    transform(-1); transform(0); transform(1);
    asm volatile("s_waitcnt lgkmcnt(0)" ::: "memory");
    for (int it = 0; it < nit; ++it) {
      __builtin_amdgcn_s_barrier();
      issue(it + 3, it + 2);
      asm volatile("s_waitcnt vmcnt(%0)" :: "n"(KDMA) : "memory");
      const unsigned da = sd_a + dslot(it);
      const unsigned xa = sx_a + xslot(it + ty - 1);
      const bool mul_ = !SX || G.is_row(ccm);
      if constexpr (SX) G.adv(ccm);
      if (mul_) {
      Frags fa, fb;
      read_frags(da, xa, 0, fa);
      read_frags(da, xa, 1, fb);
      wait_frags(fa, 1); mfma6(fa);
      read_frags(da, xa, 2, fa);
      wait_frags(fb, 1); mfma6(fb);
      read_frags(da, xa, 3, fb);
      wait_frags(fa, 1); mfma6(fa);
      wait_frags(fb, 0); mfma6(fb);
      }
      transform(it + 2);
      asm volatile("s_waitcnt lgkmcnt(0)" ::: "memory");
    }
  }
  asm volatile("s_waitcnt vmcnt(0)\n\ts_waitcnt lgkmcnt(0)" ::: "memory");
  __syncthreads();
  float* red = reinterpret_cast<float*>(smem);
  if (pgx > 0) {
#pragma unroll
    for (int j = 0; j < 6; ++j)
#pragma unroll
      for (int i = 0; i < 16; ++i) red[((rem * 6 + j) * 16 + i) * 64 + lane] = acc[j][i];
  }
  __syncthreads();
  if (pgx == 0) {
#pragma unroll
    for (int h = 0; h < 2; ++h) {
      float* part = p.scratch + (size_t)(h * p.gx + (int)blockIdx.x) * 9 * 32 * C;
#pragma unroll
      for (int j = 0; j < 3; ++j)
#pragma unroll
        for (int i = 0; i < 16; ++i) {
          const float v = acc[h * 3 + j][i] + red[((rem * 6 + h * 3 + j) * 16 + i) * 64 + lane];
          const int co = (i & 3) + 8 * (i >> 2) + 4 * (lane >> 5);
          part[((ty * 3 + j) * 32 + co) * C + cih * 32 + (lane & 31)] = v;
        }
    }
  }
}
template <bool BN> __global__ __launch_bounds__(768) void wgrad_rows64(const WgtK p) { if (p.sx) wgrad_rows64_body<BN, true>(p); else wgrad_rows64_body<BN, false>(p); }
template <bool BN> __global__ __launch_bounds__(768) void wgrad_rows64_g(const WgtKG g) {
  const WgtK& p = g.k[blockIdx.z];
  if ((int)blockIdx.x >= p.gx) return;
  if (p.sx) wgrad_rows64_body<BN, true>(p); else wgrad_rows64_body<BN, false>(p);
}

#include "wgrad_rowsx.inc"

template <int W>
__global__ __launch_bounds__(768) void wgrad_img(const WgK p) {
  constexpr int PC = 512, PXB = 128, SLACK = 18 * PXB;
  extern __shared__ __attribute__((aligned(16))) unsigned char smem[];
  unsigned char* sX = smem + SLACK;
  unsigned char* sD = sX + PC * PXB + SLACK;
  const int tid = threadIdx.x, lane = tid & 63;
  const int wv = __builtin_amdgcn_readfirstlane(tid >> 6);
  const int ty = wv >> 2, coh = (wv >> 1) & 1, cih = wv & 1;
  int b = blockIdx.x;
  const int ti = b % p.nti; b /= p.nti;
  const int tc = b % p.ntc; b /= p.ntc;
  const int chunk = b;
  const int co0 = tc * 64, ci0 = ti * 64;
  const unsigned cbytes = (unsigned)(p.C * 2), obytes = (unsigned)(p.Cout * 2);
  const __amdgpu_buffer_rsrc_t rx = make_rsrc(p.a, (unsigned)((size_t)p.M * p.C * 2)), rd = make_rsrc(p.dy, (unsigned)((size_t)p.M * p.Cout * 2));
  {
    const unsigned gch = (unsigned)(((lane & 7) ^ (((lane >> 4) & 1) << 2)) * 16);
    const unsigned pix0 = (unsigned)(chunk * PC + (lane >> 3));
#pragma unroll
    for (int k = 0; k < 11; ++k) {
      const int q = k * 12 + wv, pb = q >> 1;
      if (q >= 2 * (PC / 8)) { const unsigned z = 0u, off = 0x80000000u; asm volatile("buffer_store_dword %0, %1, %2, 0 offen" :: "v"(z), "v"(off), "s"(rd) : "memory"); }
      else if (!(q & 1)) __builtin_amdgcn_raw_ptr_buffer_load_lds(rx, (lds_void_p)(sX + pb * 1024), 16, (pix0 + (unsigned)(pb * 8)) * cbytes + (unsigned)(ci0 * 2) + gch, 0, 0, 0);
      else __builtin_amdgcn_raw_ptr_buffer_load_lds(rd, (lds_void_p)(sD + pb * 1024), 16, (pix0 + (unsigned)(pb * 8)) * obytes + (unsigned)(co0 * 2) + gch, 0, 0, 0);
    }
  }
  const unsigned sx_a = (unsigned)(size_t)(lds_void_p)sX, sd_a = (unsigned)(size_t)(lds_void_p)sD;
  const int li = lane & 15, g = lane >> 4;
  const int q4 = li >> 2, pp = li & 3;
  const int chan = 16 * (g & 1) + 4 * pp;
  const int kh = g >> 1;
  const int hrow = 8 * kh + q4;
  auto off_of = [&](int pix, int ch) {
    return pix * PXB + ((((ch >> 3)) ^ (((pix >> 1) & 1) << 2)) * 16) + (ch & 7) * 2;
  };
  const unsigned dyo = sd_a + (unsigned)off_of(hrow, coh * 32 + chan);
  unsigned xo[3];
#pragma unroll
  for (int tx = 0; tx < 3; ++tx) xo[tx] = (unsigned)((int)sx_a + off_of(hrow + (ty - 1) * W + (tx - 1), cih * 32 + chan));
  const bool row_start = (W == 8) || kh == 0, row_end = (W == 8) || kh == 1;
  const unsigned m_l = row_start ? 0xffff0000u : 0xffffffffu;
  const unsigned m_r = row_end ? 0x0000ffffu : 0xffffffffu;

  f32x16 acc[3];
#pragma unroll
  for (int j = 0; j < 3; ++j)
#pragma unroll
    for (int i = 0; i < 16; ++i) acc[j][i] = 0.f;
  struct Frags { s16x4 d0, d1, x0[3], x1[3]; };
  auto read_frags = [&](int ks, Frags& f) {
    const unsigned dk = dyo + (unsigned)(ks * 16 * PXB);
    const unsigned x0a = xo[0] + (unsigned)(ks * 16 * PXB), x1a = xo[1] + (unsigned)(ks * 16 * PXB), x2a = xo[2] + (unsigned)(ks * 16 * PXB);
    asm volatile("ds_read_b64_tr_b16 %0, %8\n\tds_read_b64_tr_b16 %1, %8 offset:512\n\t"
                 "ds_read_b64_tr_b16 %2, %9\n\tds_read_b64_tr_b16 %3, %9 offset:512\n\t"
                 "ds_read_b64_tr_b16 %4, %10\n\tds_read_b64_tr_b16 %5, %10 offset:512\n\t"
                 "ds_read_b64_tr_b16 %6, %11\n\tds_read_b64_tr_b16 %7, %11 offset:512"
                 : "=&v"(f.d0), "=&v"(f.d1), "=&v"(f.x0[0]), "=&v"(f.x1[0]), "=&v"(f.x0[1]), "=&v"(f.x1[1]), "=&v"(f.x0[2]), "=&v"(f.x1[2])
                 : "v"(dk), "v"(x0a), "v"(x1a), "v"(x2a) : "memory");
  };
  auto wait_frags = [&](Frags& f, int pending) {
    if (pending) asm volatile("s_waitcnt lgkmcnt(8)" : "+v"(f.d0), "+v"(f.d1), "+v"(f.x0[0]), "+v"(f.x1[0]), "+v"(f.x0[1]), "+v"(f.x1[1]), "+v"(f.x0[2]), "+v"(f.x1[2]) :: "memory");
    else asm volatile("s_waitcnt lgkmcnt(0)" : "+v"(f.d0), "+v"(f.d1), "+v"(f.x0[0]), "+v"(f.x1[0]), "+v"(f.x0[1]), "+v"(f.x1[1]), "+v"(f.x0[2]), "+v"(f.x1[2]) :: "memory");
  };
  typedef __attribute__((ext_vector_type(8))) short s16x8;
  typedef __attribute__((ext_vector_type(2))) unsigned u32x2;
  auto mfma3 = [&](const Frags& f, int ks) {
    const int h = (W == 8) ? ((2 * ks + kh) & 7) : (ks & 15);
    const bool rows_ok = !((ty == 0 && h == 0) || (ty == 2 && h == W - 1));
    const unsigned rm = rows_ok ? 0xffffffffu : 0u;
    const s16x8 fd = {f.d0[0], f.d0[1], f.d0[2], f.d0[3], f.d1[0], f.d1[1], f.d1[2], f.d1[3]};
#pragma unroll
    for (int j = 0; j < 3; ++j) {
      u32x2 a = __builtin_bit_cast(u32x2, f.x0[j]), c = __builtin_bit_cast(u32x2, f.x1[j]);
      a[0] &= rm & (j == 0 ? m_l : 0xffffffffu); a[1] &= rm;
      c[0] &= rm; c[1] &= rm & (j == 2 ? m_r : 0xffffffffu);
      const s16x4 xa = __builtin_bit_cast(s16x4, a), xc = __builtin_bit_cast(s16x4, c);
      const s16x8 fx = {xa[0], xa[1], xa[2], xa[3], xc[0], xc[1], xc[2], xc[3]};
      acc[j] = __builtin_amdgcn_mfma_f32_32x32x16_bf16(__builtin_bit_cast(bf16x8, fd), __builtin_bit_cast(bf16x8, fx), acc[j], 0, 0, 0);
    }
  };
#pragma unroll
  for (int sg = 0; sg < 4; ++sg) {
    if (sg == 0) asm volatile("s_waitcnt vmcnt(7)" ::: "memory");
    else if (sg == 1) asm volatile("s_waitcnt vmcnt(5)" ::: "memory");
    else if (sg == 2) asm volatile("s_waitcnt vmcnt(2)" ::: "memory");
    else asm volatile("s_waitcnt vmcnt(0)" ::: "memory");
    __builtin_amdgcn_s_barrier();
    Frags fa, fb;
    read_frags(8 * sg, fa);
#pragma unroll
    for (int k2 = 0; k2 < 8; k2 += 2) {
      const int ks = 8 * sg + k2;
      read_frags(ks + 1, fb);
      wait_frags(fa, 1); mfma3(fa, ks);
      if (k2 + 2 < 8) read_frags(ks + 2, fa);
      if (k2 + 2 < 8) wait_frags(fb, 1); else wait_frags(fb, 0);
      mfma3(fb, ks + 1);
    }
  }
  const bool ow = p.ksplit == 1 && p.overwrite && *p.overwrite != 0;
  const int ci = ci0 + cih * 32 + (lane & 31);
#pragma unroll
  for (int j = 0; j < 3; ++j)
#pragma unroll
    for (int i = 0; i < 16; ++i) {
      const int co = co0 + coh * 32 + (i & 3) + 8 * (i >> 2) + 4 * (lane >> 5);
      const size_t idx = ((size_t)(ty * 3 + j) * p.Cout + co) * p.C + ci;
      if (p.ksplit > 1) p.slabs[(size_t)chunk * 9 * p.Cout * p.C + idx] = acc[j][i];
      else if (ow) p.dw[idx] = acc[j][i];
      else p.dw[idx] += acc[j][i];
    }
}

template <int W>
__global__ __launch_bounds__(768) void wgrad_imgs(const WgK p) {
  constexpr int PC = 512, PXB = 64, SLACK = 18 * PXB, TILE = PC * PXB, STAGE = 2 * SLACK + 2 * TILE;
  extern __shared__ __attribute__((aligned(16))) unsigned char smem[];
  const int tid = threadIdx.x, lane = tid & 63;
  const int wv = __builtin_amdgcn_readfirstlane(tid >> 6);
  const int ty = wv >> 2, kq = wv & 3;
  const int ti = (int)blockIdx.x % p.nti, tc = (int)blockIdx.x / p.nti;
  const int co0 = tc * 32, ci0 = ti * 32;
  const int nch = p.ksplit;
  const unsigned cbytes = (unsigned)(p.C * 2), obytes = (unsigned)(p.Cout * 2);
  const __amdgpu_buffer_rsrc_t rx = make_rsrc(p.a, (unsigned)((size_t)p.M * p.C * 2)), rd = make_rsrc(p.dy, (unsigned)((size_t)p.M * p.Cout * 2));
  const unsigned srcx = (unsigned)(lane >> 2) * cbytes + (unsigned)(ci0 * 2 + (lane & 3) * 16);
  const unsigned srcd = (unsigned)(lane >> 2) * obytes + (unsigned)(co0 * 2 + (lane & 3) * 16);
  auto issue = [&](int c, int st) {
    unsigned char* sX = smem + st * STAGE + SLACK;
    unsigned char* sD = sX + TILE + SLACK;
    const unsigned pix0 = (unsigned)(c * PC);
#pragma unroll
    for (int k = 0; k < 6; ++k) {
      const int q = k * 12 + wv, pb = q >> 1;
      if (q >= 2 * (PC / 16)) { const unsigned z = 0u, off = 0x80000000u; asm volatile("buffer_store_dword %0, %1, %2, 0 offen" :: "v"(z), "v"(off), "s"(rd) : "memory"); }
      else if (!(q & 1)) __builtin_amdgcn_raw_ptr_buffer_load_lds(rx, (lds_void_p)(sX + pb * 1024), 16, (pix0 + (unsigned)(pb * 16)) * cbytes + srcx, 0, 0, 0);
      else __builtin_amdgcn_raw_ptr_buffer_load_lds(rd, (lds_void_p)(sD + pb * 1024), 16, (pix0 + (unsigned)(pb * 16)) * obytes + srcd, 0, 0, 0);
    }
  };
  issue(0, 0);
  if (nch > 1) issue(1, 1);

  const unsigned s_a = (unsigned)(size_t)(lds_void_p)smem;
  const int li = lane & 15, g = lane >> 4;
  const int q4 = li >> 2, pp = li & 3;
  const int kh = g >> 1;
  const int hrow = 8 * kh + q4;
  const int chb = 32 * (g & 1) + 8 * pp;
  const unsigned dyo = (unsigned)(2 * SLACK + TILE + (kq * 128 + hrow) * PXB + chb);
  unsigned xo[3];
#pragma unroll
  for (int tx = 0; tx < 3; ++tx) xo[tx] = (unsigned)(SLACK + (kq * 128 + hrow + (ty - 1) * W + (tx - 1)) * PXB + chb);
  const unsigned m_l = (W == 8 || kh == 0) ? 0xffff0000u : 0xffffffffu;
  const unsigned m_r = (W == 8 || kh == 1) ? 0x0000ffffu : 0xffffffffu;

  f32x16 acc[3];
#pragma unroll
  for (int j = 0; j < 3; ++j)
#pragma unroll
    for (int i = 0; i < 16; ++i) acc[j][i] = 0.f;

  struct Frags { s16x4 d0, d1, x0[3], x1[3]; };
  auto read_frags = [&](unsigned base, int k, Frags& f) {
    const unsigned dk = base + dyo + (unsigned)(k * 16 * PXB);
    const unsigned x0a = base + xo[0] + (unsigned)(k * 16 * PXB), x1a = base + xo[1] + (unsigned)(k * 16 * PXB), x2a = base + xo[2] + (unsigned)(k * 16 * PXB);
    asm volatile("ds_read_b64_tr_b16 %0, %8\n\tds_read_b64_tr_b16 %1, %8 offset:256\n\t"
                 "ds_read_b64_tr_b16 %2, %9\n\tds_read_b64_tr_b16 %3, %9 offset:256\n\t"
                 "ds_read_b64_tr_b16 %4, %10\n\tds_read_b64_tr_b16 %5, %10 offset:256\n\t"
                 "ds_read_b64_tr_b16 %6, %11\n\tds_read_b64_tr_b16 %7, %11 offset:256"
                 : "=&v"(f.d0), "=&v"(f.d1), "=&v"(f.x0[0]), "=&v"(f.x1[0]), "=&v"(f.x0[1]), "=&v"(f.x1[1]), "=&v"(f.x0[2]), "=&v"(f.x1[2])
                 : "v"(dk), "v"(x0a), "v"(x1a), "v"(x2a) : "memory");
  };
  auto wait_frags = [&](Frags& f, int pending) {
    if (pending) asm volatile("s_waitcnt lgkmcnt(8)" : "+v"(f.d0), "+v"(f.d1), "+v"(f.x0[0]), "+v"(f.x1[0]), "+v"(f.x0[1]), "+v"(f.x1[1]), "+v"(f.x0[2]), "+v"(f.x1[2]) :: "memory");
    else asm volatile("s_waitcnt lgkmcnt(0)" : "+v"(f.d0), "+v"(f.d1), "+v"(f.x0[0]), "+v"(f.x1[0]), "+v"(f.x0[1]), "+v"(f.x1[1]), "+v"(f.x0[2]), "+v"(f.x1[2]) :: "memory");
  };
  typedef __attribute__((ext_vector_type(8))) short s16x8;
  typedef __attribute__((ext_vector_type(2))) unsigned u32x2;
  auto mfma3 = [&](const Frags& f, int k) {
    const int h = (W == 8) ? ((2 * (8 * kq + k) + kh) & 7) : ((8 * kq + k) & 15);
    const bool rows_ok = !((ty == 0 && h == 0) || (ty == 2 && h == W - 1));
    const unsigned rm = rows_ok ? 0xffffffffu : 0u;
    const s16x8 fd = {f.d0[0], f.d0[1], f.d0[2], f.d0[3], f.d1[0], f.d1[1], f.d1[2], f.d1[3]};
#pragma unroll
    for (int j = 0; j < 3; ++j) {
      u32x2 a = __builtin_bit_cast(u32x2, f.x0[j]), c = __builtin_bit_cast(u32x2, f.x1[j]);
      a[0] &= rm & (j == 0 ? m_l : 0xffffffffu); a[1] &= rm;
      c[0] &= rm; c[1] &= rm & (j == 2 ? m_r : 0xffffffffu);
      const s16x4 xa = __builtin_bit_cast(s16x4, a), xc = __builtin_bit_cast(s16x4, c);
      const s16x8 fx = {xa[0], xa[1], xa[2], xa[3], xc[0], xc[1], xc[2], xc[3]};
      acc[j] = __builtin_amdgcn_mfma_f32_32x32x16_bf16(__builtin_bit_cast(bf16x8, fd), __builtin_bit_cast(bf16x8, fx), acc[j], 0, 0, 0);
    }
  };

  for (int c = 0; c < nch; ++c) {
    if (c + 1 < nch) asm volatile("s_waitcnt vmcnt(6)" ::: "memory");
    else asm volatile("s_waitcnt vmcnt(0)" ::: "memory");
    __builtin_amdgcn_s_barrier();
    const unsigned base = s_a + (unsigned)((c & 1) * STAGE);
    Frags fa, fb;
    read_frags(base, 0, fa);
#pragma unroll
    for (int k2 = 0; k2 < 8; k2 += 2) {
      read_frags(base, k2 + 1, fb);
      wait_frags(fa, 1); mfma3(fa, k2);
      if (k2 + 2 < 8) read_frags(base, k2 + 2, fa);
      if (k2 + 2 < 8) wait_frags(fb, 1); else wait_frags(fb, 0);
      mfma3(fb, k2 + 1);
    }
    if (c + 2 < nch) {
      __builtin_amdgcn_s_barrier();
      issue(c + 2, c & 1);
    }
  }
  __syncthreads();
  float* red = reinterpret_cast<float*>(smem);
#pragma unroll
  for (int j = 0; j < 3; ++j)
#pragma unroll
    for (int i = 0; i < 16; ++i) red[(((kq * 3 + ty) * 3 + j) * 16 + i) * 64 + lane] = acc[j][i];
  __syncthreads();
  const bool ow = p.overwrite && *p.overwrite != 0;
#pragma unroll
  for (int r = 0; r < 3; ++r) {
    const int o4 = tid + 768 * r;
    const int tap = o4 >> 8, col = (o4 >> 3) & 31, c4 = (o4 & 7) * 4;
    const int i = (col & 3) + 4 * (col >> 3), lh = (col >> 2) & 1;
    const float* src = red + (tap * 16 + i) * 64 + lh * 32 + c4;
    f32x4 v = *reinterpret_cast<const f32x4*>(src);
#pragma unroll
    for (int q = 1; q < 4; ++q) v += *reinterpret_cast<const f32x4*>(src + q * 9 * 16 * 64);
    float* dst = p.dw + ((size_t)tap * p.Cout + co0 + col) * p.C + ci0 + c4;
    if (!ow) v += *reinterpret_cast<const f32x4*>(dst);
    *reinterpret_cast<f32x4*>(dst) = v;
  }
}

constexpr int TAPS_RED_COLS = 64;
__device__ __forceinline__ void wgrad_taps_reduce_body(const float* __restrict__ scratch, float* __restrict__ dw, int CC, int gx, int vblock, int overwrite = 0) {
  __shared__ float4 sh[256];
  const int total4 = 9 * CC * CC / 4;
  const int el = threadIdx.x & 63, sl = threadIdx.x >> 6;
  const int e4 = vblock * TAPS_RED_COLS + el;
  float4 s = make_float4(0.f, 0.f, 0.f, 0.f);
  auto add4 = [](float4& a, const float4 b) { a.x += b.x; a.y += b.y; a.z += b.z; a.w += b.w; };
  if (e4 < total4) {
    const int e = e4 * 4;
    const int tap = e / (CC * CC), r = e - tap * CC * CC, co = r / CC, ci = r - co * CC;
    const float* src = scratch + ((size_t)(co >> 5) * gx * 9 + tap) * 32 * CC + (co & 31) * CC + ci;
    const size_t pstride = (size_t)9 * 32 * CC;
    int b = sl;
    for (; b + 28 < gx; b += 32) {
      float4 v[8];
#pragma unroll
      for (int u = 0; u < 8; ++u) v[u] = *reinterpret_cast<const float4*>(src + (size_t)(b + 4 * u) * pstride);
      float4 a = v[0], c = v[4];
      add4(a, v[1]); add4(c, v[5]); add4(a, v[2]); add4(c, v[6]); add4(a, v[3]); add4(c, v[7]);
      add4(a, c); add4(s, a);
    }
    for (; b < gx; b += 4) add4(s, *reinterpret_cast<const float4*>(src + (size_t)b * pstride));
  }
  sh[threadIdx.x] = s;
  __syncthreads();
  if (sl == 0 && e4 < total4) {
    float4 t = sh[el];
    add4(t, sh[64 + el]); add4(t, sh[128 + el]); add4(t, sh[192 + el]);
    float4* d = reinterpret_cast<float4*>(dw + (size_t)e4 * 4);
    float4 o = make_float4(0.f, 0.f, 0.f, 0.f);
    if (!overwrite) o = *d;
    add4(o, t);
    *d = o;
  }
}

__global__ __launch_bounds__(256) void wgrad_taps_reduce(const float* __restrict__ scratch, float* __restrict__ dw, int CC, int gx) {
  wgrad_taps_reduce_body(scratch, dw, CC, gx, (int)blockIdx.x);
}

struct WgGroupCapture {
  int n;
  int kind[RUA_MAX_WGRAD_GROUP];
  unsigned gx[RUA_MAX_WGRAD_GROUP]; int smem[RUA_MAX_WGRAD_GROUP];
  WgK g[RUA_MAX_WGRAD_GROUP]; WgdK d[RUA_MAX_WGRAD_GROUP]; WgtK t[RUA_MAX_WGRAD_GROUP];
  int post[RUA_MAX_WGRAD_GROUP];
  const float* part[RUA_MAX_WGRAD_GROUP]; float* dw[RUA_MAX_WGRAD_GROUP]; long long ndw[RUA_MAX_WGRAD_GROUP]; int parts[RUA_MAX_WGRAD_GROUP], CC[RUA_MAX_WGRAD_GROUP], rblocks[RUA_MAX_WGRAD_GROUP];
};
static thread_local WgGroupCapture* g_wg_group = nullptr;

static bool launch_rows32(int kind, bool grouped, dim3 grid, int smem, hipStream_t st, const WgtK* one, const WgtKG* many) {
  static RuaPerDevFlag attr_[18];
  bool& attr = attr_[(kind - 4) * 2 + (grouped ? 1 : 0)].get();
#define RUA_ROWS_GO(NPG_, BN_) do { \
    if (grouped) { if (!attr) { (void)hipFuncSetAttribute(reinterpret_cast<const void*>(&wgrad_rows32_g<NPG_, BN_>), hipFuncAttributeMaxDynamicSharedMemorySize, 160 * 1024); attr = true; } \
                   hipLaunchKernelGGL((wgrad_rows32_g<NPG_, BN_>), grid, dim3(NPG_ * 192), smem, st, *many); } \
    else { if (!attr) { (void)hipFuncSetAttribute(reinterpret_cast<const void*>(&wgrad_rows32<NPG_, BN_>), hipFuncAttributeMaxDynamicSharedMemorySize, 160 * 1024); attr = true; } \
           hipLaunchKernelGGL((wgrad_rows32<NPG_, BN_>), grid, dim3(NPG_ * 192), smem, st, *one); } } while (0)
#define RUA_ROWS64_GO(BN_) do { \
    if (grouped) { if (!attr) { (void)hipFuncSetAttribute(reinterpret_cast<const void*>(&wgrad_rows64_g<BN_>), hipFuncAttributeMaxDynamicSharedMemorySize, 160 * 1024); attr = true; } \
                   hipLaunchKernelGGL((wgrad_rows64_g<BN_>), grid, dim3(768), smem, st, *many); } \
    else { if (!attr) { (void)hipFuncSetAttribute(reinterpret_cast<const void*>(&wgrad_rows64<BN_>), hipFuncAttributeMaxDynamicSharedMemorySize, 160 * 1024); attr = true; } \
           hipLaunchKernelGGL((wgrad_rows64<BN_>), grid, dim3(768), smem, st, *one); } } while (0)
#define RUA_ROWSX_GO(MODE_) do { \
    if (grouped) { if (!attr) { (void)hipFuncSetAttribute(reinterpret_cast<const void*>(&wgrad_rowsx_g<MODE_>), hipFuncAttributeMaxDynamicSharedMemorySize, 160 * 1024); attr = true; } \
                   hipLaunchKernelGGL((wgrad_rowsx_g<MODE_>), grid, dim3(768), smem, st, *many); } \
    else { if (!attr) { (void)hipFuncSetAttribute(reinterpret_cast<const void*>(&wgrad_rowsx<MODE_>), hipFuncAttributeMaxDynamicSharedMemorySize, 160 * 1024); attr = true; } \
           hipLaunchKernelGGL((wgrad_rowsx<MODE_>), grid, dim3(768), smem, st, *one); } } while (0)
  switch (kind) {
    case 4: RUA_ROWS_GO(4, true); break;
    case 5: RUA_ROWS_GO(4, false); break;
    case 6: RUA_ROWS_GO(2, true); break;
    case 7: RUA_ROWS_GO(2, false); break;
    case 8: RUA_ROWS64_GO(true); break;
    case 9: RUA_ROWS64_GO(false); break;
    case 11: RUA_ROWSX_GO(0); break;
    case 12: RUA_ROWSX_GO(1); break;
    default: rua_set_error("launch_rows32: no kernel of kind %d", kind); return false;
  }
#undef RUA_ROWSX_GO
#undef RUA_ROWS64_GO
#undef RUA_ROWS_GO
  return true;
}

static int launch_wgrad_taps(const rua_wgrad_desc* d, hipStream_t st) {
  const int CC = d->C;
  WgtK k;
  k.a = (const unsigned char*)d->a; k.dy = (const unsigned char*)d->dy; k.scratch = (float*)d->workspace; k.dw = d->dw;
  k.H = d->H; k.W = d->W; k.N = d->N; k.dil = d->dil;
  k.in_scale = d->in_scale; k.in_shift = d->in_shift; k.in_relu = d->in_relu; k.sx = 0;
  const long long M = (long long)d->N * d->H * d->W;
  if (CC == 256 || CC == 128) {
    const int ncu_ = rua_cu_count();
    const int gy_ = CC == 256 ? 8 : 2;
    const int share_ = (g_tune.wgrad_taps_share && d->group_members > 1) ? d->group_members : 1;
    int gx_ = ncu_ / share_ / gy_;
    if (gx_ > ncu_ / (CC / 32)) gx_ = ncu_ / (CC / 32);
    const long long U_ = (long long)(CC == 256 ? d->N / 2 : d->N) * (d->H + d->dil);
    if (gx_ > U_ / 4) gx_ = (int)(U_ / 4);
    if (gx_ < 1) gx_ = 1;
    k.NPG = 1; k.strips = 1; k.halo = 0; k.halo4 = 0; k.group_bytes = 0; k.nchains = 0; k.spc = 0; k.seglen = 0; k.njobs = 0; k.jpw = 0;
    k.gx = gx_; k.nworkers = gx_;
    k.abytes = (unsigned)((size_t)M * CC * 2); k.dybytes = k.abytes;
    const size_t smem_ = (size_t)32 * 256 + 5 * (size_t)96 * 256 + 3 * (size_t)64 * 128;
    const int rblocks_ = rua_div_up(9 * CC * CC / 4, TAPS_RED_COLS);
    const int kd_ = CC == 256 ? 12 : 11;
    note_pending(1, gx_, (long long)9 * CC * CC, (const float*)k.scratch, d->dw, CC, rblocks_);
    if (g_wgrad_dry) return RUA_OK;
    if (g_wg_group && (g_tune.wgrad_group & 4) && g_wg_group->n < RUA_MAX_WGRAD_GROUP) {
      WgGroupCapture& c = *g_wg_group; const int i = c.n++;
      c.kind[i] = kd_; c.gx[i] = gx_; c.smem[i] = (int)smem_; c.t[i] = k;
      c.post[i] = d->defer ? 0 : 1; c.part[i] = k.scratch; c.dw[i] = d->dw; c.CC[i] = CC; c.parts[i] = gx_; c.rblocks[i] = rblocks_; c.ndw[i] = 0;
// ... 334 lines not shown
static int64_t wg_taps_bytes(const rua_wgrad_desc* d) { return (int64_t)rua_cu_count() * 9 * 32 * (int64_t)d->C * 4; }

static bool pick_wgrad_pw(const rua_wgrad_desc* d) {
  const int on = g_tune.wgrad_pw;
  auto pow2 = [](int v) { return v > 0 && (v & (v - 1)) == 0; };
  const long long M = (long long)d->N * d->H * d->W;
  const bool dense = d->stride == 1 && d->Hs == d->H && d->Ws == d->W;
  return on && d->dtype == RUA_BF16 && d->taps == 1 && d->C <= 64 && d->Cout <= 64 && d->C % 8 == 0 && d->Cout % 8 == 0 &&
         (dense || (pow2(d->H) && pow2(d->W))) && M >= 2048 && d->workspace &&
         d->workspace_bytes >= WG_PW_TAIL && M * d->Cout * 2 < (1ll << 31) &&
         (long long)d->N * d->Hs * d->Ws * d->C * 2 < (1ll << 31) &&
         (long long)(d->H - 1) * d->stride < d->Hs && (long long)(d->W - 1) * d->stride < d->Ws;
}

static int launch_wgrad_pw(const rua_wgrad_desc* d, hipStream_t st) {
  WgpK k;
  k.a = (const unsigned char*)d->a; k.dy = (const unsigned char*)d->dy; k.dw = d->dw;
  char* tail = (char*)d->workspace + d->workspace_bytes - WG_PW_TAIL;
  k.rep = (float*)tail; k.cnt = (int*)(tail + WG_PW_TAIL - 8192);
  k.C = d->C; k.Cout = d->Cout; k.Hs = d->Hs; k.Ws = d->Ws; k.H = d->H; k.W = d->W; k.stride = d->stride;
  k.dense = (d->stride == 1 && d->Hs == d->H && d->Ws == d->W) ? 1 : 0;
  int ws = 0, hs = 0; while ((1 << ws) < d->W) ++ws; while ((1 << hs) < d->H) ++hs;
  k.wshift = ws; k.hshift = hs;
  k.M = (int)((long long)d->N * d->H * d->W);
  k.abytes = (unsigned)((size_t)d->N * d->Hs * d->Ws * d->C * 2); k.dybytes = (unsigned)((size_t)k.M * d->Cout * 2);
  const int nco = d->Cout > 32 ? 2 : 1, nci = d->C > 32 ? 2 : 1;
  const int pxw = (nco + nci <= 2) ? 32 : 16;
  const int target = g_tune.wgpw_blocks > 0 ? g_tune.wgpw_blocks : rua_cu_count();
  long long waves = (long long)target * 16;
  if (waves > k.M / 128) waves = k.M / 128;
  if (waves < 16) waves = 16;
  long long ppw = (k.M + waves - 1) / waves;
  ppw = (ppw + 2 * pxw - 1) / (2 * pxw) * (2 * pxw);
  k.px_per_wave = (int)ppw;
  {
    const long long nblk = (k.M + ppw * 16 - 1) / (ppw * 16);
    k.R = (int)(nblk / 32); if (k.R < 1) k.R = 1; if (k.R > WG_PW_REPLICAS) k.R = WG_PW_REPLICAS;
    if (g_tune.wgpw_r > 0) k.R = g_tune.wgpw_r > WG_PW_REPLICAS ? WG_PW_REPLICAS : g_tune.wgpw_r;
  }
  const unsigned grid = (unsigned)((k.M + ppw * 16 - 1) / (ppw * 16));
  k.nblk = (int)grid;
  const long long nel = (long long)d->Cout * d->C;
  const bool slab = (g_tune.wgrad_pw & 2) && (d->defer || (g_tune.wgrad_pw & 4)) && (long long)grid * nel * 4 <= (long long)d->workspace_bytes - WG_PW_TAIL;
  k.slabs = slab ? (float*)d->workspace : nullptr;
  if (slab) note_pending(2, (int)grid, nel, k.slabs, d->dw, 0, (int)((nel / 4 + SLAB_RED_COLS - 1) / SLAB_RED_COLS));
  if (g_wgrad_dry) return RUA_OK;
  if (g_wg_pw && g_wg_pw->n < RUA_MAX_BRANCH) {
    WgPwCapture& c = *g_wg_pw; const int i = c.n++;
    c.k[i] = k; c.form[i] = (nco - 1) * 2 + (nci - 1); c.post[i] = (slab && !d->defer) ? 1 : 0;
    return RUA_OK;
  }
  constexpr int s11 = wgrad_pw_smem<1, 1>(), s21 = wgrad_pw_smem<2, 1>(), s12 = wgrad_pw_smem<1, 2>(), s22 = wgrad_pw_smem<2, 2>();
  static RuaPerDevFlag attr_;
  bool& attr = attr_.get();
  if (!attr) {
    (void)hipFuncSetAttribute(reinterpret_cast<const void*>(&wgrad_pw<2, 1>), hipFuncAttributeMaxDynamicSharedMemorySize, s21);
    (void)hipFuncSetAttribute(reinterpret_cast<const void*>(&wgrad_pw<1, 2>), hipFuncAttributeMaxDynamicSharedMemorySize, s12);
    (void)hipFuncSetAttribute(reinterpret_cast<const void*>(&wgrad_pw<2, 2>), hipFuncAttributeMaxDynamicSharedMemorySize, s22);
    attr = true;
  }
  if (nco == 1 && nci == 1) hipLaunchKernelGGL((wgrad_pw<1, 1>), dim3(grid), dim3(1024), s11, st, k);
  else if (nco == 2 && nci == 1) hipLaunchKernelGGL((wgrad_pw<2, 1>), dim3(grid), dim3(1024), s21, st, k);
  else if (nco == 1 && nci == 2) hipLaunchKernelGGL((wgrad_pw<1, 2>), dim3(grid), dim3(1024), s12, st, k);
  else hipLaunchKernelGGL((wgrad_pw<2, 2>), dim3(grid), dim3(1024), s22, st, k);
  RUA_LAUNCH_CHECK("wgrad_pw");
  if (slab && !d->defer) { rua_record_mid_event(st); return launch_slab_reduce(k.slabs, d->dw, nel, (int)grid, st); }
  return RUA_OK;
}

extern "C" int64_t rua_wgrad_workspace_bytes(const rua_wgrad_desc* d) {
  if (!d) return 0;
  int64_t slabs = (int64_t)64 * d->taps * d->Cout * d->C * 4;
  if (slabs > (64ll << 20)) slabs = 64ll << 20;
  const int64_t taps = wg_taps_bytes(d);
  return (taps > slabs ? taps : slabs) + WG_PW_TAIL;
}

static int slab_capacity(const rua_wgrad_desc* d, long long ndw) {
  if (!d->workspace || d->workspace_bytes <= WG_PW_TAIL) return 1;
  const long long n = (d->workspace_bytes - WG_PW_TAIL) / (ndw * 4);
  return n > 64 ? 64 : (int)n;
}

static int launch_wgrad_dmap(const rua_wgrad_desc* d, hipStream_t st) {
  WgdK k;
  k.a = (const unsigned char*)d->a; k.dy = (const unsigned char*)d->dy; k.dw = d->dw;
  k.C = d->C; k.Cout = d->Cout; k.H = d->H; k.W = d->W; k.dil = d->dil; k.taps = d->taps;
  k.M = (long long)d->N * d->H * d->W;
  int wsh = 0; while ((1 << wsh) < d->W) ++wsh;
  k.wsh = wsh;
  k.ntc = d->Cout / 128; k.nti = d->C / 128;
  const long long tiles = (long long)k.ntc * k.nti * d->taps;
  const int stages = (int)((k.M + 63) / 64);
  const int target = g_tune.wgd_blocks > 0 ? g_tune.wgd_blocks : rua_cu_count();
  long long want = target / tiles; if (want < 1) want = 1;
  if (want > stages / 4) want = stages / 4;
  if (want < 1) want = 1;
  const long long ndw = (long long)d->taps * d->Cout * d->C;
  const int cap = g_tune.wgrad_slabs ? slab_capacity(d, ndw) : 0;
  if (cap >= 2 && want > cap) want = cap;
  k.stages_per_split = (int)((stages + want - 1) / want);
  k.ksplit = (stages + k.stages_per_split - 1) / k.stages_per_split;
  k.slabs = (cap >= 2 && k.ksplit > 1) ? (float*)d->workspace : nullptr;
  k.abytes = (unsigned)((size_t)k.M * d->C * 2); k.dybytes = (unsigned)((size_t)k.M * d->Cout * 2);
  k.ks_slow = g_tune.wgd_ks_slow;
  if (k.slabs) note_pending(2, k.ksplit, ndw, k.slabs, d->dw, 0, (int)((ndw / 4 + SLAB_RED_COLS - 1) / SLAB_RED_COLS));
  if (g_wgrad_dry) return RUA_OK;
  if (g_wg_group && (g_tune.wgrad_group & 8) && g_wg_group->n < RUA_MAX_WGRAD_GROUP) {
    WgGroupCapture& c = *g_wg_group; const int i = c.n++;
    c.kind[i] = 3; c.gx[i] = (unsigned)(tiles * k.ksplit); c.smem[i] = 96 * 1024; c.d[i] = k;
    c.post[i] = (k.slabs && !d->defer) ? 2 : 0; c.part[i] = k.slabs; c.dw[i] = d->dw; c.ndw[i] = ndw; c.parts[i] = k.ksplit; c.CC[i] = 0; c.rblocks[i] = 0;
    return RUA_OK;
  }
  static RuaPerDevFlag attr_;
  bool& attr = attr_.get();
  if (!attr) { (void)hipFuncSetAttribute(reinterpret_cast<const void*>(&wgrad_dmap), hipFuncAttributeMaxDynamicSharedMemorySize, 96 * 1024); attr = true; }
  hipLaunchKernelGGL(wgrad_dmap, dim3((unsigned)(tiles * k.ksplit)), dim3(256), 96 * 1024, st, k);
  RUA_LAUNCH_CHECK("wgrad_dmap");
  if (k.slabs && !d->defer) { rua_record_mid_event(st); return launch_slab_reduce(k.slabs, d->dw, ndw, k.ksplit, st); }
  return RUA_OK;
}

static bool wgrad_rows256_ok(const rua_wgrad_desc* d) {
  return (g_tune.wgrad_rows & 32) && d->dtype == RUA_BF16 && d->taps == 9 && d->stride == 1 && d->C == 256 && d->Cout == 256 && d->W == 32 && d->N % 2 == 0 && d->N >= 2 &&
         d->Hs == d->H && d->Ws == d->W && d->dil >= 1 && d->dil <= 16 && !d->in_scale && d->workspace && d->workspace_bytes >= wg_taps_bytes(d) &&
         (long long)d->N * d->H * d->W * d->C * 2 < (1ll << 31);
}
extern "C" int rua_wgrad_kind(const rua_wgrad_desc* d) {
  if (!d) return RUA_ERR_ARG;
  if (pick_wgrad_pw(d)) return 3;
  {
    const int on = g_tune.wgrad_dmap;
    auto pow2 = [](int v) { return v > 0 && (v & (v - 1)) == 0; };
    if (on && !wgrad_rows256_ok(d) && d->dtype == RUA_BF16 && (d->taps == 9 || d->taps == 1) && d->stride == 1 && d->C % 128 == 0 && d->Cout % 128 == 0 &&
        d->Hs == d->H && d->Ws == d->W && pow2(d->H) && pow2(d->W) && d->dil >= 1 &&
        ((long long)d->N * d->H * d->W + 64 * 64) * (d->C > d->Cout ? d->C : d->Cout) * 2 < (1ll << 31)) {
      const long long tiles = (long long)d->taps * (d->Cout / 128) * (d->C / 128);
      const long long stages = ((long long)d->N * d->H * d->W + 63) / 64;
      const int mint = g_tune.wgd_mintiles;
      if (on == 2 || (tiles >= mint && tiles <= 64 && stages >= 64)) return 2;
    }
  }
  const bool rows128 = (g_tune.wgrad_rows & 4) && d->C == 128 && d->W == 64 && !d->in_scale;
  if (wgrad_rows256_ok(d)) return 1;
  const bool ok = d->dtype == RUA_BF16 && d->taps == 9 && d->stride == 1 && d->C == d->Cout && (d->C == 32 || d->C == 64 || rows128) &&
                  d->W % 64 == 0 && d->Hs == d->H && d->Ws == d->W && d->dil >= 1 && d->dil <= 31 && d->workspace &&
                  d->workspace_bytes >= wg_taps_bytes(d) && (long long)d->N * d->H * d->W * d->C * 2 < (1ll << 31);
  return ok ? 1 : 0;
}

static int wgrad_img_pick(const rua_wgrad_desc* d) {
  const long long M = (long long)d->N * d->H * d->W;
  if (!((g_tune.wgrad_rows & 8) && d->dtype == RUA_BF16 && d->taps == 9 && d->stride == 1 && d->dil == 1 && d->Hs == d->H && d->Ws == d->W && d->H == d->W &&
        (d->W == 8 || d->W == 16) && d->C % 32 == 0 && d->Cout % 32 == 0 && M % 512 == 0 && !d->in_scale)) return 0;
  if ((g_tune.wgrad_rows & 16) && M >= 1024 && (long long)(d->C / 32) * (d->Cout / 32) >= rua_cu_count() / 2) return 2;
  if (d->C % 64 || d->Cout % 64) return 0;
  if (M == 512 || (g_tune.wgrad_slabs && slab_capacity(d, (long long)9 * d->Cout * d->C) >= (int)(M / 512))) return 1;
  return 0;
}
extern "C" int rua_wgrad_img_kind(const rua_wgrad_desc* d) { return (d && rua_wgrad_kind(d) == 0) ? wgrad_img_pick(d) : 0; }

struct WgBatchMember { long long want; WgK k; unsigned grid; long long ndw; };
static thread_local WgBatchMember* g_wg_batch = nullptr;

extern "C" int rua_conv_wgrad(const rua_wgrad_desc* d, void* stream) {
  RUA_CHECK_ARG(d && d->a && d->dy && d->dw, "rua_conv_wgrad: null pointer");
  RUA_CHECK_ARG(d->dtype == RUA_F32 || d->dtype == RUA_BF16, "rua_conv_wgrad: bad dtype");
  const int vec = d->dtype == RUA_BF16 ? 8 : 4;
  RUA_CHECK_ARG(d->C % vec == 0 && d->Cout % vec == 0, "rua_conv_wgrad: C=%d Cout=%d must be multiples of %d", d->C, d->Cout, vec);
  RUA_CHECK_ARG(d->taps == 1 || d->taps == 9, "rua_conv_wgrad: taps must be 1 or 9");
  if (rua_wgrad_kind(d) == 1) return launch_wgrad_taps(d, (hipStream_t)stream);
  RUA_CHECK_ARG(d->in_scale == nullptr, "rua_conv_wgrad: in_scale / in_shift (normalise on load) needs the all-taps kernel (rua_wgrad_kind() == 1)");
  if (rua_wgrad_kind(d) == 2) return launch_wgrad_dmap(d, (hipStream_t)stream);
  if (rua_wgrad_kind(d) == 3) return launch_wgrad_pw(d, (hipStream_t)stream);
  RUA_CHECK_ARG((long long)(d->H - 1) * d->stride < d->Hs && (long long)(d->W - 1) * d->stride < d->Ws,
                "rua_conv_wgrad: input %dx%d too small for gradient %dx%d stride %d", d->Hs, d->Ws, d->H, d->W, d->stride);
  WgK k;
  k.a = (const unsigned char*)d->a; k.dy = (const unsigned char*)d->dy; k.dw = d->dw; k.overwrite = d->overwrite_dev;
  k.C = d->C; k.Hs = d->Hs; k.Ws = d->Ws; k.Cout = d->Cout; k.H = d->H; k.W = d->W; k.N = d->N;
  k.stride = d->stride; k.dil = d->dil; k.taps = d->taps;
  k.M = (long long)d->N * d->H * d->W;
  RUA_CHECK_ARG(k.M * d->Cout * 4 < (1ll << 31) && (long long)d->N * d->Hs * d->Ws * d->C * 4 < (1ll << 31),
                "rua_conv_wgrad: tensors must stay below 2 GiB (32-bit offsets)");
  auto lg2 = [](int v) { int s = 0; while ((1 << s) < v) ++s; return (1 << s) == v ? s : -1; };
  k.wshift = lg2(d->W); k.hshift = lg2(d->H);
  if (k.wshift < 0 || k.hshift < 0) k.wshift = k.hshift = -1;
  k.ntc = (d->Cout + 63) / 64; k.nti = (d->C + 63) / 64;
  const int img_kind = wgrad_img_pick(d);
  if (img_kind) {
    hipStream_t st_ = (hipStream_t)stream;
    const long long ndw_ = (long long)9 * d->Cout * d->C;
    if (img_kind == 2) {
      if (g_wgrad_dry) return RUA_OK;
      k.ksplit = (int)(k.M / 512); k.pix_per_block = 512; k.slabs = nullptr;
      k.nti = d->C / 32; k.ntc = d->Cout / 32;
      constexpr int smems_ = 4 * 9 * 16 * 64 * 4;
      static RuaPerDevFlag attrs_;
      bool& attrs = attrs_.get();
      if (!attrs) {
        (void)hipFuncSetAttribute(reinterpret_cast<const void*>(&wgrad_imgs<8>), hipFuncAttributeMaxDynamicSharedMemorySize, 160 * 1024);
        (void)hipFuncSetAttribute(reinterpret_cast<const void*>(&wgrad_imgs<16>), hipFuncAttributeMaxDynamicSharedMemorySize, 160 * 1024);
        attrs = true;
      }
      if (d->W == 8) hipLaunchKernelGGL(wgrad_imgs<8>, dim3((unsigned)(k.nti * k.ntc)), dim3(768), smems_, st_, k);
      else hipLaunchKernelGGL(wgrad_imgs<16>, dim3((unsigned)(k.nti * k.ntc)), dim3(768), smems_, st_, k);
      RUA_LAUNCH_CHECK("wgrad_imgs");
      return RUA_OK;
    }
    k.ksplit = (int)(k.M / 512);
    k.pix_per_block = 512;
    k.slabs = k.ksplit > 1 ? (float*)d->workspace : nullptr;
    if (k.slabs) note_pending(2, k.ksplit, ndw_, k.slabs, d->dw, 0, (int)((ndw_ / 4 + SLAB_RED_COLS - 1) / SLAB_RED_COLS));
    if (g_wgrad_dry) return RUA_OK;
    const unsigned grid_ = (unsigned)(k.ntc * k.nti * k.ksplit);
    constexpr int smem_ = 2 * 512 * 128 + 2 * 18 * 128;
    static RuaPerDevFlag attr_;
    bool& attr = attr_.get();
    if (!attr) {
      (void)hipFuncSetAttribute(reinterpret_cast<const void*>(&wgrad_img<8>), hipFuncAttributeMaxDynamicSharedMemorySize, 160 * 1024);
      (void)hipFuncSetAttribute(reinterpret_cast<const void*>(&wgrad_img<16>), hipFuncAttributeMaxDynamicSharedMemorySize, 160 * 1024);
      attr = true;
    }
    if (d->W == 8) hipLaunchKernelGGL(wgrad_img<8>, dim3(grid_), dim3(768), smem_, st_, k);
    else hipLaunchKernelGGL(wgrad_img<16>, dim3(grid_), dim3(768), smem_, st_, k);
    RUA_LAUNCH_CHECK("wgrad_img");
    if (k.slabs && !d->defer) { rua_record_mid_event(st_); return launch_slab_reduce(k.slabs, d->dw, ndw_, k.ksplit, st_); }
    return RUA_OK;
  }
  const long long tiles = (long long)k.ntc * k.nti * d->taps;
  const int target = (g_tune.wgrad_blocks > 0 ? g_tune.wgrad_blocks : 2 * rua_cu_count());
  long long want = target / tiles; if (want < 1) want = 1;
  long long stages = (k.M + 63) / 64;
  if (g_wg_batch && g_wg_batch->want > 0) want = g_wg_batch->want;
  if (want > stages) want = stages;
  const long long ndw = (long long)d->taps * d->Cout * d->C;
  const int cap = (g_tune.wgrad_slabs && ndw % 4 == 0) ? slab_capacity(d, ndw) : 0;
  if (cap >= 2 && want > cap) want = cap;
  long long spb = (stages + want - 1) / want;
  k.pix_per_block = (int)(spb * 64);
  k.ksplit = (int)((k.M + k.pix_per_block - 1) / k.pix_per_block);
  k.slabs = (cap >= 2 && k.ksplit > 1) ? (float*)d->workspace : nullptr;
  const long long grid = tiles * k.ksplit;
  RUA_CHECK_ARG(grid < (1ll << 31), "rua_conv_wgrad: grid too large");
  hipStream_t st = (hipStream_t)stream;
  if (k.slabs) note_pending(2, k.ksplit, ndw, k.slabs, d->dw, 0, (int)((ndw / 4 + SLAB_RED_COLS - 1) / SLAB_RED_COLS));
  if (g_wgrad_dry) return RUA_OK;
  if (g_wg_batch) { g_wg_batch->k = k; g_wg_batch->grid = (unsigned)grid; g_wg_batch->ndw = ndw; return RUA_OK; }
  if (g_wg_group && (g_tune.wgrad_group & 1) && g_wg_group->n < RUA_MAX_WGRAD_GROUP && d->dtype == RUA_BF16) {
    WgGroupCapture& c = *g_wg_group; const int i = c.n++;
    c.kind[i] = 0; c.gx[i] = (unsigned)grid; c.smem[i] = 0; c.g[i] = k;
    c.post[i] = (k.slabs && !d->defer) ? 2 : 0; c.part[i] = k.slabs; c.dw[i] = d->dw; c.ndw[i] = ndw; c.parts[i] = k.ksplit; c.CC[i] = 0; c.rblocks[i] = 0;
    return RUA_OK;
  }
  if (d->dtype == RUA_BF16) hipLaunchKernelGGL((wgrad_kernel<bf16_t>), dim3((unsigned)grid), dim3(256), 0, st, k);
  else hipLaunchKernelGGL((wgrad_kernel<float>), dim3((unsigned)grid), dim3(256), 0, st, k);
  RUA_LAUNCH_CHECK("wgrad_kernel");
  if (k.slabs && !d->defer) { rua_record_mid_event(st); return launch_slab_reduce(k.slabs, d->dw, ndw, k.ksplit, st); }
  return RUA_OK;
}

static thread_local int g_wg_group_last_grids = 0;
extern "C" int rua_wgrad_group_last_grids(void) { return g_wg_group_last_grids; }

constexpr int WG_BATCH_MAX_MEMBERS = 4 * RUA_MAX_WGRAD_BATCH;
static bool wgrad_batch_ok(const rua_wgrad_desc* d, int n) {
  if (!(g_tune.wgrad_group & 1) || n > WG_BATCH_MAX_MEMBERS) return false;
  for (int i = 0; i < n; ++i) {
    if (!d[i].a || !d[i].dy || !d[i].dw || d[i].dtype != RUA_BF16 || !d[i].batch || d[i].in_scale) return false;
    if (d[i].C <= 0 || d[i].Cout <= 0 || d[i].C % 8 || d[i].Cout % 8 || (d[i].taps != 1 && d[i].taps != 9)) return false;
    if (rua_wgrad_kind(d + i) != 0 || wgrad_img_pick(d + i) != 0) return false;
  }
  for (int i = 0; i < n; ++i)
    for (int j = i + 1; j < n; ++j) if (d[i].dw == d[j].dw) return false;
  return true;
}
static void wgrad_batch_split(const rua_wgrad_desc* d, int n, long long* want) {
  long long work = 0;
  for (int i = 0; i < n; ++i)
    work += (((long long)d[i].N * d[i].H * d[i].W + 63) / 64) * ((d[i].Cout + 63) / 64) * ((d[i].C + 63) / 64) * d[i].taps;
  const long long budget = g_tune.wgrad_batch_blocks > 0 ? g_tune.wgrad_batch_blocks : 4ll * rua_cu_count();
  for (int i = 0; i < n; ++i) {
    const long long stages = ((long long)d[i].N * d[i].H * d[i].W + 63) / 64;
    long long w = work > 0 ? (budget * stages + work / 2) / work : 1;
    want[i] = (g_tune.wgrad_group & 32) ? 0 : (w < 1 ? 1 : w);
  }
}
static int wgrad_batch_members(const rua_wgrad_desc* d, int n, WgBatchMember* mem, rua_wgrad_pending* recs, bool dry) {
  long long want[RUA_MAX_WGRAD_BATCH];
  wgrad_batch_split(d, n, want);
  int rc = RUA_OK;
  for (int i = 0; i < n && rc == RUA_OK; ++i) {
    mem[i].want = want[i]; mem[i].grid = 0;
    if (recs) { memset(recs + i, 0, sizeof(*recs)); g_wgrad_pending = recs + i; }
    g_wg_batch = mem + i; g_wgrad_dry = dry;
    rc = rua_conv_wgrad(d + i, nullptr);
    g_wg_batch = nullptr; g_wgrad_dry = false; g_wgrad_pending = nullptr;
    if (recs) recs[i].overwrite_dev = d[i].overwrite_dev;
  }
  return rc;
}
static int wgrad_batch_launch(const rua_wgrad_desc* d, int n, hipStream_t st) {
  int grids = 0;
  for (int base = 0; base < n; base += RUA_MAX_WGRAD_BATCH) {
    const int m = n - base < RUA_MAX_WGRAD_BATCH ? n - base : RUA_MAX_WGRAD_BATCH;
    WgBatchMember mem[RUA_MAX_WGRAD_BATCH];
    const int rc = wgrad_batch_members(d + base, m, mem, nullptr, false);
    if (rc != RUA_OK) return rc;
    int order[RUA_MAX_WGRAD_BATCH];
    for (int i = 0; i < m; ++i) order[i] = i;
    for (int i = 1; i < m; ++i) {
      const int o = order[i]; int j = i;
      while (j > 0 && mem[order[j - 1]].k.pix_per_block < mem[o].k.pix_per_block) { order[j] = order[j - 1]; --j; }
      order[j] = o;
    }
    WgKB g;
    unsigned long long total = 0;
    for (int i = 0; i < m; ++i) { g.k[i] = mem[order[i]].k; total += mem[order[i]].grid; g.end[i] = (unsigned)total; }
    for (int i = m; i < RUA_MAX_WGRAD_BATCH; ++i) { g.k[i] = g.k[0]; g.end[i] = (unsigned)total; }
    g.n = m;
    RUA_CHECK_ARG(total >= 1 && total < (1ull << 31), "rua_conv_wgrad_group: grid too large");
    hipLaunchKernelGGL(wgrad_kernel_b, dim3((unsigned)total), dim3(256), 0, st, g);
    RUA_LAUNCH_CHECK("wgrad_kernel_b");
    ++grids;
    for (int i = 0; i < m; ++i)
      if (mem[i].k.slabs && !d[base + i].defer) { const int rr = launch_slab_reduce(mem[i].k.slabs, mem[i].k.dw, mem[i].ndw, mem[i].k.ksplit, st); if (rr != RUA_OK) return rr; }
  }
  g_wg_group_last_grids = grids;
  return RUA_OK;
}
extern "C" int rua_wgrad_group_plan(const rua_wgrad_desc* d, int n, rua_wgrad_pending* out) {
  RUA_CHECK_ARG(d && out && n >= 1, "rua_wgrad_group_plan: bad arguments");
  if (!wgrad_batch_ok(d, n)) {
    for (int i = 0; i < n; ++i) { const int rc = rua_wgrad_plan(d + i, out + i); if (rc != RUA_OK) return rc; }
    return RUA_OK;
  }
  for (int base = 0; base < n; base += RUA_MAX_WGRAD_BATCH) {
    const int m = n - base < RUA_MAX_WGRAD_BATCH ? n - base : RUA_MAX_WGRAD_BATCH;
    WgBatchMember mem[RUA_MAX_WGRAD_BATCH];
    const int rc = wgrad_batch_members(d + base, m, mem, out + base, true);
    if (rc != RUA_OK) return rc;
  }
  return RUA_OK;
}
extern "C" int rua_conv_wgrad_group(const rua_wgrad_desc* d, int n, void* stream) {
  RUA_CHECK_ARG(d && n >= 1, "rua_conv_wgrad_group: no members");
  hipStream_t st = (hipStream_t)stream;
  if (wgrad_batch_ok(d, n)) {
    static thread_local rua_wgrad_pending recs[WG_BATCH_MAX_MEMBERS];
    const int rp = rua_wgrad_group_plan(d, n, recs);
    if (rp != RUA_OK) return rp;
    bool overlap = false;
    for (int i = 0; i < n && !overlap; ++i)
      for (int j = i + 1; j < n && !overlap; ++j) {
        if (recs[i].kind != 2 || recs[j].kind != 2) continue;
        const float* a0 = recs[i].partials; const float* b0 = recs[j].partials;
        overlap = a0 < b0 + (long long)recs[j].parts * recs[j].n && b0 < a0 + (long long)recs[i].parts * recs[i].n;
      }
    if (!overlap) return wgrad_batch_launch(d, n, st);
    g_wg_group_last_grids = n;
    for (int i = 0; i < n; ++i) { const int rc = rua_conv_wgrad(d + i, stream); if (rc != RUA_OK) return rc; }
    return RUA_OK;
  }
  RUA_CHECK_ARG(n <= RUA_MAX_WGRAD_GROUP, "rua_conv_wgrad_group: 1..%d members (more only in the batched form)", RUA_MAX_WGRAD_GROUP);
  bool shared = false;
  for (int i = 0; i < n; ++i)
    for (int j = i + 1; j < n; ++j) {
      const char* a0 = (const char*)d[i].workspace; const char* b0 = (const char*)d[j].workspace;
      if (a0 && b0 && a0 < b0 + d[j].workspace_bytes && b0 < a0 + d[i].workspace_bytes) shared = true;
      if (d[i].dw == d[j].dw) shared = true;
    }
  g_wg_group_last_grids = n;
  {
    bool allpw = n >= 2 && (g_tune.wgrad_group & 16);
    for (int i = 0; i < n && allpw; ++i) allpw = rua_wgrad_kind(d + i) == 3;
    for (int i = 0; i < n && allpw; ++i)
      for (int j = i + 1; j < n; ++j) {
        const char* ti = (const char*)d[i].workspace + d[i].workspace_bytes - WG_PW_TAIL; const char* tj = (const char*)d[j].workspace + d[j].workspace_bytes - WG_PW_TAIL;
// ... 134 lines not shown
```

resunet_a_mltsk_keras_amd/engine.py:

```python
from __future__ import annotations

import ctypes as C
import math
import os
from dataclasses import dataclass, field
from typing import Dict, List, Optional, Tuple

import numpy as np
import torch

from . import _lib as L
from .scenes import MAP_HEADS, AffineSceneBatch, SceneBatch, check_radius, check_tolerance, check_views, view_rows

BN_EPS, BN_MOMENTUM, KERAS_EPS = 1e-3, 0.99, 1e-7
HEADS = ["seg", "bound", "dist", "color"]
SUMS_REPLICAS = 1


@dataclass
class ModelConfig:
    input_shape: Tuple[int, int, int] = (256, 256, 3)
    num_classes: int = 5
    multitasking: bool = False
    variant: str = "model2"
# ... 370 lines not shown
        if self.training:
            d.stats, d.replicas = stats.ptr, stats.R
        d.count, d.bessel_n, d.momentum, d.eps = float(count), float(bessel or count), BN_MOMENTUM, BN_EPS
        for i, (bn, c, o) in enumerate(zip(bns, coefs, outs)):
            b = d.br[i]
            b.gamma, b.beta, b.moving_mean, b.moving_var = self.P(bn["gamma"]), self.P(bn["beta"]), self.S(bn["mm"]), self.S(bn["mv"])
            b.scale, b.shift, b.mean, b.rstd, b.out = c.scale, c.shift, c.mean, c.rstd, o.ptr
            if out_stats and self.training and not relu and not self.dry and self.e.bn_out_stats:
                o.stats = Stat(self.salloc(2 * x.C), 1)
                b.out_stats = o.stats.ptr
        plan.keep += coefs
        if defer is not None:
            defer.append(d)
            return outs, coefs
        self.issue(plan, [d], "rua_bn_fwd")
        return outs, coefs

    def issue(self, plan: Plan, descs: List, one: str, group: Optional[str] = None):
        grads = [o for d in descs for o in getattr(d, "grads", ())]
        if len(descs) == 1:
            plan.keep.append(descs[0])
            plan.add(one, C.byref(descs[0]), grads=grads)
        elif descs:
            arr = (type(descs[0]) * len(descs))(*descs)
            plan.keep.append(arr)
            plan.add(group, arr, len(descs), grads=grads)

    def bn_fwd_group(self, plan: Plan, items: List[tuple], relu: bool, count):
        ds, outs, coefs = [], [], []
        for x, bn, st in items:
            o, c = self.bn_fwd(plan, x, [bn], relu, st, count, defer=ds)
            outs.append(o[0]); coefs.append(c[0])
        self.issue(plan, ds, "rua_bn_fwd", "rua_bn_fwd_group")
        return outs, coefs

    def bn_coefs(self, plan: Plan, like: Ten, bns: List[dict], stats: List[Optional[Stat]], count, bessel=None) -> List[Coef]:
        coefs = [Coef(self, bn["C"]) for bn in bns]
        d = L.BnFwdDesc()
        d.x, d.M, d.C, d.dtype, d.nb, d.relu = None, like.M, like.C, self.dt, len(bns), 1
        d.training = 1 if self.training else 0
        d.count, d.bessel_n, d.momentum, d.eps = float(count), float(bessel or count), BN_MOMENTUM, BN_EPS
        for i, (bn, c, st) in enumerate(zip(bns, coefs, stats)):
            b = d.br[i]
            b.gamma, b.beta, b.moving_mean, b.moving_var = self.P(bn["gamma"]), self.P(bn["beta"]), self.S(bn["mm"]), self.S(bn["mv"])
            b.scale, b.shift, b.mean, b.rstd, b.out = c.scale, c.shift, c.mean, c.rstd, None
            if self.training:
                b.stats, b.replicas = st.ptr, st.R
        plan.keep += [d] + coefs
        plan.add("rua_bn_fwd", C.byref(d))
        return coefs

    def bn_bwd(self, plan: Plan, gs: List[Ten], coefs: List[Coef], bns: List[dict], stats2: List[Stat], x: Ten, out: Ten,
               accumulate: int, count, dskip: Optional[Ten] = None, masked=False, skip_bias: Optional[List[int]] = None, defer: Optional[List] = None,
               dx_bias: bool = False, stats2_out: Optional[List[bool]] = None):
        d = L.BnBwdDesc()
        d.x, d.dx, d.M, d.C, d.dtype, d.nb = x.ptr, out.ptr, x.M, x.C, self.dt, len(gs)
        d.dskip = dskip.ptr if dskip is not None else None
        d.masked, d.accumulate, d.count = 1 if masked else 0, accumulate, float(count)
        for i, (g, c, bn, s2) in enumerate(zip(gs, coefs, bns, stats2)):
            b = d.br[i]
            b.g, b.stats2, b.replicas = g.ptr, s2.ptr, s2.R
            b.stats2_out = 1 if (stats2_out and stats2_out[i]) else 0
            b.gamma, b.mean, b.rstd, b.scale, b.shift = self.P(bn["gamma"]), c.mean, c.rstd, c.scale, c.shift
            b.dgamma, b.dbeta = self.G(bn["gamma"]), self.G(bn["beta"])
        d.grads = [o for bn in bns for o in (bn["gamma"], bn["beta"])]
        st = None
        cg = x.C // self.vec
        if skip_bias and dskip is not None and not (cg <= 256 and 256 % cg == 0):
            self.bias_grad(plan, dskip, skip_bias)
            skip_bias = None
        if skip_bias and dskip is not None:
            blocks = max(1, min(1024, x.M * (x.C // self.vec) // 256))
            st = self.stat(x.C, blocks, burst=True)
            d.skip_stats, d.skip_replicas = st.ptr, st.R
        if defer is not None:
            assert st is None
            defer.append(d)
            return
        sx = None
        if (dx_bias and x.bn_src is not None and not x.bn_src["fused"] and not accumulate and not self.dry and self.e.bn_dx_bias and cg <= 256 and 256 % cg == 0):
            blocks = max(1, min(1024, x.M * (x.C // self.vec) // 256))
            s2 = self.stat(x.C, blocks, burst=True)
            d.dx_stats, d.dx_replicas = s2.ptr, s2.R
            x.bn_src["s2"], x.bn_src["s2_out"] = s2, True
            x.bias_done = True
        elif (dx_bias and x.bias_offs and not accumulate and not self.dry and self.e.bn_dx_bias and cg <= 256 and 256 % cg == 0):
            blocks = max(1, min(1024, x.M * (x.C // self.vec) // 256))
            sx = self.stat(x.C, blocks, burst=True)
            d.dx_stats, d.dx_replicas = sx.ptr, sx.R
            x.bias_done = True
        self.issue(plan, [d], "rua_bn_bwd")
        if st is not None:
            self.stats_to_grads(plan, st, x.C, skip_bias)
        if sx is not None:
            self.stats_to_grads(plan, sx, x.C, x.bias_offs)

    def bn_bwd_group(self, plan: Plan, items: List[tuple]):
        ds: List = []
        for g, c, bn, s2, x, out, cnt in items:
            self.bn_bwd(plan, [g], [c], [bn], [s2], x, out, 0, cnt, defer=ds)
        self.issue(plan, ds, "rua_bn_bwd", "rua_bn_bwd_group")

    def conv(self, plan: Plan, segs, layer_segs, cout, bias_ptr, out: Ten, stride=1, residual: Optional[Ten] = None,
             out_relu=False, stats=None, bias_more=(), in_bn: Optional["Coef"] = None, accumulate: int = 0, in_fold=None):
        d = self.conv_desc(segs, layer_segs, cout, bias_ptr, out, stride, residual, out_relu, stats, bias_more, in_bn, accumulate, in_fold)
        plan.keep.append(d)
        plan.add("rua_conv_fwd", C.byref(d))

    def bn_fold(self, plan: Plan, bn: dict, stats: Stat, count, bessel=None):
        c = Coef(self, bn["C"])
        f = L.BnFold()
        f.stats, f.replicas = stats.ptr, stats.R
        f.count, f.bessel_n, f.eps, f.momentum = float(count), float(bessel or count), BN_EPS, BN_MOMENTUM
        f.gamma, f.beta, f.moving_mean, f.moving_var = self.P(bn["gamma"]), self.P(bn["beta"]), self.S(bn["mm"]), self.S(bn["mv"])
        f.scale, f.shift, f.mean, f.rstd = c.scale, c.shift, c.mean, c.rstd
        plan.keep += [c, f]
        return c, f

    def conv_desc(self, segs, layer_segs, cout, bias_ptr, out: Ten, stride=1, residual=None, out_relu=False, stats=None, bias_more=(),
                  in_bn=None, accumulate=0, in_fold=None):
        d = L.ConvDesc()
        d.nseg = len(segs)
        for i, ((t, up, dil, taps), ps) in enumerate(zip(segs, layer_segs)):
            assert t.C == ps["C"], (t.C, ps)
            s = d.seg[i]
            s.x, s.w, s.C, s.Hs, s.Ws, s.up_shift, s.dil, s.taps = t.ptr, self.Wf(ps["dst"]), t.C, t.H, t.W, up, dil, taps
        d.N, d.H, d.W, d.Cout, d.stride, d.dtype = out.N, out.H, out.W, cout, stride, self.dt
        d.bias = bias_ptr
        for i, b in enumerate(bias_more):
            d.bias_more[i] = b
        if residual is not None:
            d.aux, d.aux_mode = residual.ptr, 1
        d.out_relu = 1 if out_relu else 0
        d.y, d.out_stride, d.OH, d.OW = out.ptr, 1, out.H, out.W
        if stats is not None:
            d.stats, d.stats_mode, d.stats_replicas = stats.ptr, 1, stats.R
        d.accumulate = accumulate
        if in_fold is not None:
            d.in_fold, d.in_relu = C.addressof(in_fold), 1
        elif in_bn is not None:
            d.in_scale, d.in_shift, d.in_relu = in_bn.scale, in_bn.shift, 1
        self._ws(d)
        return d

    def fused_input_ok(self, x: Ten, nf: int, dil: int) -> bool:
        if self.dry or self.dt != L.RUA_BF16 or not self.e.fuse_bn:
            return False
        d = L.ConvDesc()
        d.nseg = 1
        sg = d.seg[0]
        sg.x, sg.w, sg.C, sg.Hs, sg.Ws, sg.up_shift, sg.dil, sg.taps = x.ptr, x.ptr, x.C, x.H, x.W, 0, dil, 9
        d.N, d.H, d.W, d.Cout, d.stride, d.dtype = x.N, x.H, x.W, nf, 1, self.dt
        d.y, d.out_stride, d.OH, d.OW = x.ptr, 1, x.H, x.W
        w = L.WgradDesc()
        w.a, w.C, w.Hs, w.Ws, w.dy, w.Cout, w.H, w.W = x.ptr, x.C, x.H, x.W, x.ptr, nf, x.H, x.W
        w.N, w.stride, w.dil, w.taps, w.dtype = x.N, 1, dil, 9, self.dt
        sc = self.e.scratch
        w.workspace, w.workspace_bytes = sc.data_ptr(), sc.numel() * 4
        lib = L.lib()
        return lib.raw("rua_conv_fused_input_ok")(C.byref(d)) == 1 and lib.raw("rua_wgrad_kind")(C.byref(w)) == 1

    def _ws(self, d):
        if not self.dry and self.e.split_k and d.N * d.H * d.W * d.Cout * 4 <= self.e.workspace.numel() * 4:
            d.workspace, d.workspace_bytes = self.e.workspace.data_ptr(), self.e.workspace.numel() * 4

    def dgrad(self, plan: Plan, dy: Ten, wd_ptr, cin: int, dil: int, taps: int, out: Ten, accumulate: int,
              mask: Optional[Tuple[Ten, Optional[int], Optional[int]]] = None, stats2: Optional[int] = None,
              stat_aux: Optional[Ten] = None, out_stride: int = 1):
        d = self.dgrad_desc(dy, wd_ptr, cin, dil, taps, out, accumulate, mask, stats2, stat_aux, out_stride)
        plan.keep.append(d)
        plan.add("rua_conv_fwd", C.byref(d))

    def conv_group(self, plan: Plan, descs: List):
        if len(descs) > L.RUA_MAX_BRANCH:
            self.conv_group(plan, descs[:L.RUA_MAX_BRANCH])
            self.conv_group(plan, descs[L.RUA_MAX_BRANCH:])
            return
        self.issue(plan, descs, "rua_conv_fwd", "rua_conv_fwd_group")

    def conv_sum(self, plan: Plan, descs: List):
        self.issue(plan, descs, "rua_conv_fwd", "rua_conv_fwd_sum")

    def dgrad_desc(self, dy: Ten, wd_ptr, cin: int, dil: int, taps: int, out: Ten, accumulate: int, mask=None, stats2=None,
                   stat_aux=None, out_stride: int = 1):
        d = L.ConvDesc()
        d.nseg = 1
        s = d.seg[0]
        s.x, s.w, s.C, s.Hs, s.Ws, s.up_shift, s.dil, s.taps = dy.ptr, wd_ptr, dy.C, dy.H, dy.W, 0, dil, taps
        d.N, d.H, d.W, d.Cout, d.stride, d.dtype = dy.N, dy.H, dy.W, cin, 1, self.dt
        d.accumulate = accumulate
        d.y, d.out_stride, d.OH, d.OW = out.ptr, out_stride, out.H, out.W
        if mask is not None:
            d.aux, d.aux_mode, d.mscale, d.mshift = mask[0].ptr, 2, mask[1], mask[2]
        elif stat_aux is not None:
            d.aux, d.aux_mode = stat_aux.ptr, 3
        if stats2 is not None:
            d.stats, d.stats_mode, d.stats_replicas = stats2.ptr, 2, stats2.R
        self._ws(d)
        return d

    def wgrad_desc(self, plan: Plan, a: Ten, dy: Ten, dw_off: int, stride: int, dil: int, taps: int, in_bn: Optional["Coef"] = None,
                   may_flush: bool = True, group: int = 0, defer_ok: bool = True):
        d = L.WgradDesc()
        d.group_members = group
        d.a, d.C, d.Hs, d.Ws = a.ptr, a.C, a.H, a.W
        if in_bn is not None:
            d.in_scale, d.in_shift, d.in_relu = in_bn.scale, in_bn.shift, 1
        d.dy, d.Cout, d.H, d.W = dy.ptr, dy.C, dy.H, dy.W
        d.N, d.stride, d.dil, d.taps, d.dtype = dy.N, stride, dil, taps, self.dt
        if not self.dry and self.e.wgrad_overwrite:
            d.overwrite_dev = self.e.ow_flag.data_ptr()
        defer = (not self.dry) and self.e.defer_reduce and plan is self.bwd and defer_ok
        if defer and may_flush:
            bucket = self.e.dist.bucket_of(dw_off) if self.e.dist is not None else 0
            if (self.pending or self.later) and (bucket != self.pending_bucket or self.pending_bytes > self.e.flush_bytes):
                self.flush_wgrad(plan)
            self.pending_bucket = bucket
        d.dw, d.grads = self.G(dw_off), (dw_off,)
        if not self.dry:
            d.workspace, d.workspace_bytes = self.e.scratch.data_ptr(), self.e.scratch.numel() * 4
            if defer:
                self._defer_wgrad(plan, d, dw_off)
        return d

    def wgrad(self, plan: Plan, a: Ten, dy: Ten, dw_off: int, stride: int, dil: int, taps: int, in_bn: Optional["Coef"] = None):
        if not self.wgrad_later(plan, a, dy, dw_off, stride, dil, taps, in_bn):
            self.issue(plan, [self.wgrad_desc(plan, a, dy, dw_off, stride, dil, taps, in_bn)], "rua_conv_wgrad")

    def wgrad_later(self, plan: Plan, a: Ten, dy: Ten, dw_off: int, stride: int, dil: int, taps: int, in_bn: Optional["Coef"] = None) -> bool:
        if self.dry or plan is not self.bwd or in_bn is not None or self.dt != L.RUA_BF16 or not (self.e.batch_wgrad and self.e.defer_reduce):
            return False
        d = self.wgrad_desc(plan, a, dy, dw_off, stride, dil, taps, defer_ok=False)
        lib = L.lib()
        if lib.raw("rua_wgrad_kind")(C.byref(d)) != 0 or lib.raw("rua_wgrad_img_kind")(C.byref(d)) != 0:
            return False
        bucket = self.e.dist.bucket_of(dw_off) if self.e.dist is not None else 0
        if (self.pending or self.later) and (bucket != self.pending_bucket or self.pending_bytes > self.e.flush_bytes):
            self.flush_wgrad(plan)
        self.pending_bucket = bucket
        d.batch, d.defer = 1, 1
        self.later.append((d, dw_off))
        return True

    def _issue_later(self, plan: Plan):
        if not self.later:
            return
        lib = L.lib()
        n = len(self.later)
        arr = (L.WgradDesc * n)(*[d for d, _ in self.later])
        recs = (L.WgradPending * n)()
        lib.call("rua_wgrad_group_plan", arr, n, recs)
        for i in range(n):
            if recs[i].kind != 0:
                nbytes = recs[i].parts * recs[i].n * 4 + (264 << 10)
                ws = self.alloc(((nbytes + 3) // 4,), torch.float32, zero=True)
                arr[i].workspace, arr[i].workspace_bytes = ws.data_ptr(), ws.numel() * 4
                self.pending_bytes += nbytes
        first = [(recs[i].kind, recs[i].parts) for i in range(n)]
        lib.call("rua_wgrad_group_plan", arr, n, recs)
        assert first == [(recs[i].kind, recs[i].parts) for i in range(n)]
        for i, (_, off) in enumerate(self.later):
            if recs[i].kind != 0:
                self.pending.append((L.WgradPending.from_buffer_copy(recs[i]), off))
        plan.keep.append(arr)
        prev, plan.scope = plan.scope, "wgrad_batch"
        plan.add("rua_conv_wgrad_group", arr, n, grads=[off for _, off in self.later])
        plan.scope = prev
        self.later = []

    def wgrad_group(self, plan: Plan, specs: List[tuple]):
        if len(specs) == 1 or self.dry:
            for sp in specs:
                self.wgrad(plan, *sp)
            return
        if len(specs) > L.RUA_MAX_WGRAD_GROUP:
            self.wgrad_group(plan, specs[:L.RUA_MAX_WGRAD_GROUP])
            self.wgrad_group(plan, specs[L.RUA_MAX_WGRAD_GROUP:])
            return
        descs = [self.wgrad_desc(plan, *sp, may_flush=(i == 0), group=len(specs)) for i, sp in enumerate(specs)]
        self.issue(plan, descs, "rua_conv_wgrad", "rua_conv_wgrad_group")

    def wgrad_now_or_later(self, plan: Plan, specs: List[tuple]) -> List[tuple]:
        if self.dry or len(specs) < 2 or 2 * len(specs) > L.RUA_MAX_WGRAD_GROUP or specs[0][0].C not in self.e.merge_wgrad:
            self.wgrad_group(plan, specs)
            return []
        return specs

    def wgrad_pw_group(self, plan: Plan, specs: List[tuple]):
        lib = L.lib()
        if self.dry or len(specs) < 2 or self.dt != L.RUA_BF16 or not self.e.group_wgrad_pw or len(specs) > L.RUA_MAX_BRANCH:
            if len(specs) > L.RUA_MAX_BRANCH and not self.dry and self.dt == L.RUA_BF16 and self.e.group_wgrad_pw:
                self.wgrad_pw_group(plan, specs[:L.RUA_MAX_BRANCH])
                self.wgrad_pw_group(plan, specs[L.RUA_MAX_BRANCH:])
                return
            for sp in specs:
                self.wgrad(plan, *sp)
            return
        if not all(lib.raw("rua_wgrad_kind")(C.byref(self.wgrad_desc(plan, *sp, defer_ok=False))) == 3 for sp in specs):
            for sp in specs:
                self.wgrad(plan, *sp)
            return
        descs = [self.wgrad_desc(plan, *sp, may_flush=(i == 0)) for i, sp in enumerate(specs)]
        for d in descs:
            if d.defer:
                continue
            nbytes = int(lib.raw("rua_wgrad_workspace_bytes")(C.byref(d)))
            ws = self.alloc(((nbytes + 3) // 4,), torch.float32, zero=True)
            d.workspace, d.workspace_bytes = ws.data_ptr(), ws.numel() * 4
        self.issue(plan, descs, "rua_conv_wgrad", "rua_conv_wgrad_group")

    def _defer_wgrad(self, plan: Plan, d, dw_off: int):
        lib = L.lib()
        rec = L.WgradPending()
# ... 1478 lines not shown
```

Before: 1336 patches/s.

## Fuse BN-normalise-on-load into img2 conv and whole-image wgrad kernels

Extends the 8x8/16x16 image conv kernel (conv_img2) and the whole-image wgrad kernels so they apply a BatchNorm scale/shift plus ReLU to the input tile in LDS. The conv kernel can also fold the BN statistics itself. The fused-input eligibility check now accepts these kernels, so deep low-resolution layers can skip a separate BN-apply pass and the extra activation write and read that goes with it. The cost is an in-LDS transform pass with extra barriers inside the main loops and more shared memory per block.

```diff
diff --git a/include/rua_hip.h b/include/rua_hip.h
--- a/include/rua_hip.h
+++ b/include/rua_hip.h
@@ -123,6 +123,7 @@
 int rua_wgrad_group_plan(const rua_wgrad_desc* d, int n, rua_wgrad_pending* out);
 int64_t rua_wgrad_workspace_bytes(const rua_wgrad_desc* d);
 int rua_wgrad_kind(const rua_wgrad_desc* d);
+int rua_wgrad_fused_input_ok(const rua_wgrad_desc* d);
 int rua_wgrad_img_kind(const rua_wgrad_desc* d);
 
 typedef struct rua_wprep_item { int64_t src_off, dst_off; int32_t taps, Cout, C, pad; } rua_wprep_item;
diff --git a/resunet_a_mltsk_keras_amd/_lib.py b/resunet_a_mltsk_keras_amd/_lib.py
--- a/resunet_a_mltsk_keras_amd/_lib.py
+++ b/resunet_a_mltsk_keras_amd/_lib.py
@@ -111,6 +111,7 @@
     "rua_wgrad_workspace_bytes": ([C.POINTER(WgradDesc)], i64),
     "rua_wgrad_kind": ([C.POINTER(WgradDesc)], i32),
     "rua_wgrad_img_kind": ([C.POINTER(WgradDesc)], i32),
+    "rua_wgrad_fused_input_ok": ([C.POINTER(WgradDesc)], i32),
     "rua_wgrad_plan": ([C.POINTER(WgradDesc), C.POINTER(WgradPending)], i32),
     "rua_wgrad_reduce_batch": ([vp, i32, i32, vp], i32),
     "rua_weight_prep": ([vp, vp, vp, vp, i32, i32, i32, vp], i32),
diff --git a/resunet_a_mltsk_keras_amd/csrc/conv_img2.hip b/resunet_a_mltsk_keras_amd/csrc/conv_img2.hip
--- a/resunet_a_mltsk_keras_amd/csrc/conv_img2.hip
+++ b/resunet_a_mltsk_keras_amd/csrc/conv_img2.hip
@@ -4,14 +4,17 @@
   const unsigned char* x; const unsigned char* w; float* ws;
   int C, Cout, H, M, ngrp, nco, ksplit, cpb;
   unsigned xbytes, wbytes;
+  const float* in_scale; const float* in_shift; int in_relu;
+  int has_fold; rua_bn_fold f;
 };
 template <int V> struct Img2IC { static constexpr int value = V; };
 
-template <int W>
+template <int W, bool BN>
 __device__ __forceinline__ void conv_img2_body(const Img2K& q) {
   constexpr int NW = 8, HW = W * W, PXB = 256, NPX = 256;
   constexpr int XB = NPX * PXB, ZOFF = XB, SWO = XB + 256;
   constexpr int KS = 8, TAPB = 64 * PXB, WBUF = 3 * TAPB, WPW = (WBUF / 1024) / NW, XPW = (XB / 1024) / NW;
+  constexpr int TABO = SWO + WBUF, REDO = TABO + 1024;
   extern __shared__ __attribute__((aligned(16))) unsigned char smem[];
   const int tid = threadIdx.x, lane = tid & 63;
   const int wv = __builtin_amdgcn_readfirstlane(tid >> 6);
@@ -59,11 +62,81 @@
 #pragma unroll
     for (int k = 0; k < 16; ++k) acc[t][k] = 0.f;
 
+  float* tab = reinterpret_cast<float*>(smem + TABO);
+  auto load_table = [&](int ch) {
+    if constexpr (BN) {
+      const int c = tid & 127, gi = tid >> 7, cg = ch * 128 + c;
+      if (!q.has_fold) {
+        if (tid < 128) { tab[c] = q.in_scale[cg]; tab[128 + c] = q.in_shift ? q.in_shift[cg] : 0.f; }
+      } else {
+        typedef __attribute__((ext_vector_type(2))) unsigned u32x2_t;
+        constexpr int KMAX = 8;
+        double* red = reinterpret_cast<double*>(smem + REDO);
+        const __amdgpu_buffer_rsrc_t rs = make_rsrc(q.f.stats, (unsigned)((size_t)q.f.replicas * 2 * C * 8));
+        u32x2_t x[KMAX], y[KMAX];
+#pragma unroll
+        for (int k = 0; k < KMAX; ++k) {
+          const unsigned off = (unsigned)(((gi + k * 4) * 2 * C + cg) * 8);
+          x[k] = __builtin_amdgcn_raw_buffer_load_b64(rs, off, 0, 0);
+          y[k] = __builtin_amdgcn_raw_buffer_load_b64(rs, off + (unsigned)(C * 8), 0, 0);
+        }
+        float gam = 0.f, bet = 0.f;
+        if (gi == 0) { gam = q.f.gamma[cg]; bet = q.f.beta[cg]; }
+        double a1 = 0, a2 = 0;
+#pragma unroll
+        for (int k = 0; k < KMAX; ++k) { a1 += __builtin_bit_cast(double, x[k]); a2 += __builtin_bit_cast(double, y[k]); }
+        for (int r = gi + KMAX * 4; r < q.f.replicas; r += 4) { a1 += q.f.stats[(size_t)r * 2 * C + cg]; a2 += q.f.stats[(size_t)r * 2 * C + C + cg]; }
+        red[(gi * 2) * 128 + c] = a1; red[(gi * 2 + 1) * 128 + c] = a2;
+        __syncthreads();
+        if (gi == 0) {
+          double s1 = 0, s2 = 0;
+          for (int g = 0; g < 4; ++g) { s1 += red[(g * 2) * 128 + c]; s2 += red[(g * 2 + 1) * 128 + c]; }
+          const double mean = s1 / q.f.count;
+          double v = s2 / q.f.count - mean * mean;
+          if (v < 0) v = 0;
+          const double r = 1.0 / sqrt(v + (double)q.f.eps);
+          const double sc = (double)gam * r;
+          const float scf = (float)sc, shf = (float)((double)bet - mean * sc);
+          tab[c] = scf; tab[128 + c] = shf;
+          if (cs == 0 && grp == 0) {
+            q.f.scale[cg] = scf; q.f.shift[cg] = shf;
+            if (q.f.mean) q.f.mean[cg] = (float)mean;
+            if (q.f.rstd) q.f.rstd[cg] = (float)r;
+            if (q.f.moving_mean) {
+              const double unb = q.f.bessel_n > 1 ? v * (q.f.bessel_n / (q.f.bessel_n - 1)) : v;
+              q.f.moving_mean[cg] = (float)((double)q.f.moving_mean[cg] * q.f.momentum + mean * (1.0 - q.f.momentum));
+              q.f.moving_var[cg] = (float)((double)q.f.moving_var[cg] * q.f.momentum + unb * (1.0 - q.f.momentum));
+            }
+          }
+        }
+      }
+    }
+  };
+  auto transform = [&]() {
+    if constexpr (BN) {
+      const int cgp = ((tid & 15) ^ ((tid >> 4) & 15)) * 8;
+      float sc8[8], sh8[8];
+#pragma unroll
+      for (int j = 0; j < 8; ++j) { sc8[j] = tab[cgp + j]; sh8[j] = tab[128 + cgp + j]; }
+#pragma unroll
+      for (int j = 0; j < XB / 16 / 512; ++j) {
+        uint4* pc = reinterpret_cast<uint4*>(smem + (tid + 512 * j) * 16);
+        float fv[8];
+        ET<bf16_t>::unpack(*pc, fv);
+#pragma unroll
+        for (int e = 0; e < 8; ++e) { fv[e] = fmaf(sc8[e], fv[e], sh8[e]); if (q.in_relu) fv[e] = fmaxf(fv[e], 0.f); }
+        *pc = ET<bf16_t>::pack(fv);
+      }
+    }
+  };
+
   issue_x(ch0);
 #pragma unroll
   for (int i = 0; i < WPW; ++i) issue_w1(ch0, 0, i, true);
+  load_table(ch0);
   asm volatile("s_waitcnt vmcnt(0)" ::: "memory");
   __syncthreads();
+  transform();
   bf16x8 wf[3][KS];
 #pragma unroll
   for (int tx = 0; tx < 3; ++tx)
@@ -115,7 +188,13 @@
     if (ty == 2 && chl + 1 < q.cpb) {
       __builtin_amdgcn_s_barrier();
       issue_x(ch0 + chl + 1);
+      if constexpr (BN) load_table(ch0 + chl + 1);
       asm volatile("s_waitcnt vmcnt(0)" ::: "memory");
+      if constexpr (BN) {
+        __syncthreads();
+        transform();
+        asm volatile("s_waitcnt lgkmcnt(0)" ::: "memory");
+      }
     }
   }
   float* slab = q.ws + ((size_t)ks * q.M + m0) * q.Cout + co0 + coh * 32 + 8 * kh;
@@ -137,10 +216,11 @@
     }
   }
 }
-template <int W> __global__ __launch_bounds__(512) void conv_img2(const Img2K q) { conv_img2_body<W>(q); }
+template <int W, bool BN> __global__ __launch_bounds__(512) void conv_img2(const Img2K q) { conv_img2_body<W, BN>(q); }
 
 int rua_pick_img2(const rua_conv_desc* d) {
-  if (!g_tune.conv_img2 || g_conv_group || d->dtype != RUA_BF16 || d->nseg != 1 || d->in_scale || d->in_fold) return 0;
+  if (!g_tune.conv_img2 || g_conv_group || d->dtype != RUA_BF16 || d->nseg != 1) return 0;
+  if (d->in_fold && (d->in_scale || d->in_shift)) return 0;
   const rua_conv_seg& g = d->seg[0];
   if (g.taps != 9 || g.dil != 1 || d->stride != 1 || d->out_stride != 1 || g.up_shift != 0 || g.Hs != d->H || g.Ws != d->W || d->H != d->W || (d->W != 8 && d->W != 16) ||
       d->OH != d->H || d->OW != d->W) return 0;
@@ -164,17 +244,30 @@
   q.x = (const unsigned char*)g.x; q.w = (const unsigned char*)g.w; q.ws = (float*)d->workspace;
   q.C = g.C; q.Cout = d->Cout; q.H = d->H; q.M = (int)k.M; q.ngrp = (int)(k.M / 256); q.nco = d->Cout / 64; q.ksplit = KS; q.cpb = (g.C / 128) / KS;
   q.xbytes = (unsigned)((size_t)k.M * g.C * 2); q.wbytes = (unsigned)((size_t)9 * d->Cout * g.C * 2);
+  const bool bn = d->in_scale || d->in_fold;
+  q.in_scale = d->in_scale; q.in_shift = d->in_shift; q.in_relu = d->in_relu; q.has_fold = d->in_fold ? 1 : 0;
+  memset(&q.f, 0, sizeof(q.f));
+  if (d->in_fold) {
+    q.f = *d->in_fold;
+    RUA_CHECK_ARG(q.f.stats && q.f.replicas >= 1 && q.f.count > 0 && q.f.gamma && q.f.beta && q.f.scale && q.f.shift, "conv_img2: incomplete in_fold");
+    RUA_CHECK_ARG((q.f.moving_mean == nullptr) == (q.f.moving_var == nullptr), "conv_img2: in_fold needs both moving statistics or neither");
+    RUA_CHECK_ARG((size_t)q.f.replicas * 2 * g.C * 8 < 0x7FFFFF00ull, "conv_img2: in_fold statistics of 2 GiB or more");
+  }
   k.nbn = (d->Cout + 63) / 64; k.nbm = (int)(k.M / 256); k.ksplit = KS; k.stages_per_split = 0; k.ws = (float*)d->workspace; k.cnt = nullptr;
   const unsigned grid = (unsigned)(q.ngrp * q.nco * KS);
-  constexpr int smem = 256 * 256 + 256 + 3 * 64 * 256;
+  constexpr int smem = 256 * 256 + 256 + 3 * 64 * 256, smem_bn = smem + 1024 + 4 * 2 * 128 * 8;
   static RuaPerDevFlag attr;
   if (!attr.get()) {
-    (void)hipFuncSetAttribute(reinterpret_cast<const void*>(&conv_img2<8>), hipFuncAttributeMaxDynamicSharedMemorySize, smem);
-    (void)hipFuncSetAttribute(reinterpret_cast<const void*>(&conv_img2<16>), hipFuncAttributeMaxDynamicSharedMemorySize, smem);
+    (void)hipFuncSetAttribute(reinterpret_cast<const void*>(&conv_img2<8, false>), hipFuncAttributeMaxDynamicSharedMemorySize, smem);
+    (void)hipFuncSetAttribute(reinterpret_cast<const void*>(&conv_img2<16, false>), hipFuncAttributeMaxDynamicSharedMemorySize, smem);
+    (void)hipFuncSetAttribute(reinterpret_cast<const void*>(&conv_img2<8, true>), hipFuncAttributeMaxDynamicSharedMemorySize, smem_bn);
+    (void)hipFuncSetAttribute(reinterpret_cast<const void*>(&conv_img2<16, true>), hipFuncAttributeMaxDynamicSharedMemorySize, smem_bn);
     attr.get() = true;
   }
-  if (d->W == 8) hipLaunchKernelGGL((conv_img2<8>), dim3(grid), dim3(512), smem, st, q);
-  else hipLaunchKernelGGL((conv_img2<16>), dim3(grid), dim3(512), smem, st, q);
+  if (bn && d->W == 8) hipLaunchKernelGGL((conv_img2<8, true>), dim3(grid), dim3(512), smem_bn, st, q);
+  else if (bn) hipLaunchKernelGGL((conv_img2<16, true>), dim3(grid), dim3(512), smem_bn, st, q);
+  else if (d->W == 8) hipLaunchKernelGGL((conv_img2<8, false>), dim3(grid), dim3(512), smem, st, q);
+  else hipLaunchKernelGGL((conv_img2<16, false>), dim3(grid), dim3(512), smem, st, q);
   RUA_LAUNCH_CHECK("conv_img2");
   return rua_splitk_finish_bf16(k, st);
 }
diff --git a/resunet_a_mltsk_keras_amd/csrc/conv_mfma.hip b/resunet_a_mltsk_keras_amd/csrc/conv_mfma.hip
--- a/resunet_a_mltsk_keras_amd/csrc/conv_mfma.hip
+++ b/resunet_a_mltsk_keras_amd/csrc/conv_mfma.hip
@@ -1838,8 +1838,13 @@
     g_last_ksplit = 1;
     return rua_launch_conv_strip(k, d, st);
   }
-  RUA_CHECK_ARG(d->in_scale == nullptr && d->in_fold == nullptr, "rua_conv_fwd: in_scale / in_shift / in_fold (normalise on load) is not available for "
-                                        "this shape: ask rua_conv_fused_input_ok() first");
+  if (d->in_scale || d->in_fold) {
+    const int img2_ks = rua_pick_img2(d);
+    RUA_CHECK_ARG(img2_ks != 0, "rua_conv_fwd: in_scale / in_shift / in_fold (normalise on load) is not available for "
+                                "this shape: ask rua_conv_fused_input_ok() first");
+    g_last_ksplit = img2_ks;
+    return rua_launch_conv_img2(k, d, img2_ks, st);
+  }
   if (pick_halo(d)) {
     k.nbn = 1; k.nbm = 1; k.ksplit = 1; k.stages_per_split = 0; k.ws = nullptr; k.cnt = nullptr;
     g_last_ksplit = 1;
@@ -2048,7 +2053,7 @@
   if (pick_dmap(d)) return 128;
   return pick_bn(d, (long long)d->N * d->H * d->W);
 }
-extern "C" int rua_conv_fused_input_ok(const rua_conv_desc* d) { return (d && rua_pick_strip(d)) ? 1 : 0; }
+extern "C" int rua_conv_fused_input_ok(const rua_conv_desc* d) { return (d && (rua_pick_strip(d) || rua_pick_img2(d))) ? 1 : 0; }
 
 extern "C" int rua_conv_kernel_id(const rua_conv_desc* d) {
   if (!d) return RUA_ERR_ARG;
diff --git a/resunet_a_mltsk_keras_amd/csrc/conv_wgrad.hip b/resunet_a_mltsk_keras_amd/csrc/conv_wgrad.hip
--- a/resunet_a_mltsk_keras_amd/csrc/conv_wgrad.hip
+++ b/resunet_a_mltsk_keras_amd/csrc/conv_wgrad.hip
@@ -1012,10 +1012,35 @@
 
 #include "wgrad_rowsx.inc"
 
-template <int W>
-__global__ __launch_bounds__(768) void wgrad_img(const WgK p) {
+struct WgImgK { WgK k; const float* in_scale; const float* in_shift; int in_relu; };
+template <int NT>
+__device__ __forceinline__ void wgrad_img_xform(unsigned char* sX, const float* tab, int e0, int e1, int tid, int relu, int pxpieces, int swz) {
+  const unsigned xa = (unsigned)(size_t)(lds_void_p)sX, ta = (unsigned)(size_t)(lds_void_p)tab;
+  for (int e = e0 + tid; e < e1; e += NT) {
+    const int pix = e / pxpieces, ch = (((e % pxpieces) ^ (swz ? (((pix >> 1) & 1) << 2) : 0))) * 8;
+    const unsigned pa = xa + (unsigned)(e * 16), ca = ta + (unsigned)(ch * 4);
+    typedef __attribute__((ext_vector_type(4))) unsigned u32x4_t;
+    u32x4_t v; f32x4 s0, s1, h0, h1;
+    asm volatile("ds_read_b128 %0, %5\n\tds_read_b128 %1, %6\n\tds_read_b128 %2, %6 offset:16\n\tds_read_b128 %3, %6 offset:256\n\tds_read_b128 %4, %6 offset:272\n\t"
+                 "s_waitcnt lgkmcnt(0)" : "=&v"(v), "=&v"(s0), "=&v"(s1), "=&v"(h0), "=&v"(h1) : "v"(pa), "v"(ca) : "memory");
+    float f[8];
+    ET<bf16_t>::unpack(__builtin_bit_cast(uint4, v), f);
+#pragma unroll
+    for (int j = 0; j < 4; ++j) { f[j] = fmaf(s0[j], f[j], h0[j]); f[4 + j] = fmaf(s1[j], f[4 + j], h1[j]); }
+    if (relu) {
+#pragma unroll
+      for (int j = 0; j < 8; ++j) f[j] = fmaxf(f[j], 0.f);
+    }
+    v = __builtin_bit_cast(u32x4_t, ET<bf16_t>::pack(f));
+    asm volatile("ds_write_b128 %0, %1" :: "v"(pa), "v"(v) : "memory");
+  }
+}
+template <int W, bool BN>
+__global__ __launch_bounds__(768) void wgrad_img(const WgImgK pk) {
+  const WgK& p = pk.k;
   constexpr int PC = 512, PXB = 128, SLACK = 18 * PXB;
   extern __shared__ __attribute__((aligned(16))) unsigned char smem[];
+  const float* tab = reinterpret_cast<const float*>(smem + 2 * SLACK + 2 * PC * PXB);
   unsigned char* sX = smem + SLACK;
   unsigned char* sD = sX + PC * PXB + SLACK;
   const int tid = threadIdx.x, lane = tid & 63;
@@ -1031,6 +1056,12 @@
   {
     const unsigned gch = (unsigned)(((lane & 7) ^ (((lane >> 4) & 1) << 2)) * 16);
     const unsigned pix0 = (unsigned)(chunk * PC + (lane >> 3));
+    if constexpr (BN) {
+      if (wv < 2) {
+        const float* src = wv == 0 ? pk.in_scale : pk.in_shift;
+        __builtin_amdgcn_raw_ptr_buffer_load_lds(make_rsrc(src, (unsigned)(p.C * 4)), (lds_void_p)(smem + 2 * SLACK + 2 * PC * PXB + wv * 256), 4, (unsigned)((ci0 + lane) * 4), 0, 0, 0);
+      }
+    }
 #pragma unroll
     for (int k = 0; k < 11; ++k) {
       const int q = k * 12 + wv, pb = q >> 1;
@@ -1100,6 +1131,12 @@
     else if (sg == 2) asm volatile("s_waitcnt vmcnt(2)" ::: "memory");
     else asm volatile("s_waitcnt vmcnt(0)" ::: "memory");
     __builtin_amdgcn_s_barrier();
+    if constexpr (BN) {
+      const int P0 = sg == 0 ? 0 : sg == 1 ? 192 : sg == 2 ? 288 : 432, P1 = sg == 0 ? 192 : sg == 1 ? 288 : sg == 2 ? 432 : 512;
+      wgrad_img_xform<768>(sX, tab, 8 * P0, 8 * P1, tid, pk.in_relu, 8, 1);
+      asm volatile("s_waitcnt lgkmcnt(0)" ::: "memory");
+      __builtin_amdgcn_s_barrier();
+    }
     Frags fa, fb;
     read_frags(8 * sg, fa);
 #pragma unroll
@@ -1126,10 +1163,12 @@
     }
 }
 
-template <int W>
-__global__ __launch_bounds__(768) void wgrad_imgs(const WgK p) {
+template <int W, bool BN>
+__global__ __launch_bounds__(768) void wgrad_imgs(const WgImgK pk) {
+  const WgK& p = pk.k;
   constexpr int PC = 512, PXB = 64, SLACK = 18 * PXB, TILE = PC * PXB, STAGE = 2 * SLACK + 2 * TILE;
   extern __shared__ __attribute__((aligned(16))) unsigned char smem[];
+  const float* tab = reinterpret_cast<const float*>(smem + 2 * STAGE);
   const int tid = threadIdx.x, lane = tid & 63;
   const int wv = __builtin_amdgcn_readfirstlane(tid >> 6);
   const int ty = wv >> 2, kq = wv & 3;
@@ -1152,6 +1191,12 @@
       else __builtin_amdgcn_raw_ptr_buffer_load_lds(rd, (lds_void_p)(sD + pb * 1024), 16, (pix0 + (unsigned)(pb * 16)) * obytes + srcd, 0, 0, 0);
     }
   };
+  if constexpr (BN) {
+    if (wv < 2) {
+      const float* src = wv == 0 ? pk.in_scale : pk.in_shift;
+      __builtin_amdgcn_raw_ptr_buffer_load_lds(make_rsrc(src, (unsigned)(p.C * 4)), (lds_void_p)(smem + 2 * STAGE + wv * 256), 4, lane < 32 ? (unsigned)((ci0 + lane) * 4) : 0x80000000u, 0, 0, 0);
+    }
+  }
   issue(0, 0);
   if (nch > 1) issue(1, 1);
 
@@ -1211,6 +1256,11 @@
     if (c + 1 < nch) asm volatile("s_waitcnt vmcnt(6)" ::: "memory");
     else asm volatile("s_waitcnt vmcnt(0)" ::: "memory");
     __builtin_amdgcn_s_barrier();
+    if constexpr (BN) {
+      wgrad_img_xform<768>(smem + (c & 1) * STAGE + SLACK, tab, 0, TILE / 16, tid, pk.in_relu, 4, 0);
+      asm volatile("s_waitcnt lgkmcnt(0)" ::: "memory");
+      __builtin_amdgcn_s_barrier();
+    }
     const unsigned base = s_a + (unsigned)((c & 1) * STAGE);
     Frags fa, fb;
     read_frags(base, 0, fa);
@@ -1851,13 +1901,14 @@
 static int wgrad_img_pick(const rua_wgrad_desc* d) {
   const long long M = (long long)d->N * d->H * d->W;
   if (!((g_tune.wgrad_rows & 8) && d->dtype == RUA_BF16 && d->taps == 9 && d->stride == 1 && d->dil == 1 && d->Hs == d->H && d->Ws == d->W && d->H == d->W &&
-        (d->W == 8 || d->W == 16) && d->C % 32 == 0 && d->Cout % 32 == 0 && M % 512 == 0 && !d->in_scale)) return 0;
+        (d->W == 8 || d->W == 16) && d->C % 32 == 0 && d->Cout % 32 == 0 && M % 512 == 0 && (!d->in_scale || d->in_shift))) return 0;
   if ((g_tune.wgrad_rows & 16) && M >= 1024 && (long long)(d->C / 32) * (d->Cout / 32) >= rua_cu_count() / 2) return 2;
   if (d->C % 64 || d->Cout % 64) return 0;
   if (M == 512 || (g_tune.wgrad_slabs && slab_capacity(d, (long long)9 * d->Cout * d->C) >= (int)(M / 512))) return 1;
   return 0;
 }
 extern "C" int rua_wgrad_img_kind(const rua_wgrad_desc* d) { return (d && rua_wgrad_kind(d) == 0) ? wgrad_img_pick(d) : 0; }
+extern "C" int rua_wgrad_fused_input_ok(const rua_wgrad_desc* d) { return (d && (rua_wgrad_kind(d) == 1 || rua_wgrad_img_kind(d) != 0)) ? 1 : 0; }
 
 struct WgBatchMember { long long want; WgK k; unsigned grid; long long ndw; };
 static thread_local WgBatchMember* g_wg_batch = nullptr;
@@ -1869,7 +1920,8 @@
   RUA_CHECK_ARG(d->C % vec == 0 && d->Cout % vec == 0, "rua_conv_wgrad: C=%d Cout=%d must be multiples of %d", d->C, d->Cout, vec);
   RUA_CHECK_ARG(d->taps == 1 || d->taps == 9, "rua_conv_wgrad: taps must be 1 or 9");
   if (rua_wgrad_kind(d) == 1) return launch_wgrad_taps(d, (hipStream_t)stream);
-  RUA_CHECK_ARG(d->in_scale == nullptr, "rua_conv_wgrad: in_scale / in_shift (normalise on load) needs the all-taps kernel (rua_wgrad_kind() == 1)");
+  RUA_CHECK_ARG(d->in_scale == nullptr || rua_wgrad_img_kind(d) != 0, "rua_conv_wgrad: in_scale / in_shift (normalise on load) needs the all-taps kernel or a whole-image kernel "
+                                                                      "(rua_wgrad_fused_input_ok() == 1)");
   if (rua_wgrad_kind(d) == 2) return launch_wgrad_dmap(d, (hipStream_t)stream);
   if (rua_wgrad_kind(d) == 3) return launch_wgrad_pw(d, (hipStream_t)stream);
   RUA_CHECK_ARG((long long)(d->H - 1) * d->stride < d->Hs && (long long)(d->W - 1) * d->stride < d->Ws,
@@ -1897,12 +1949,18 @@
       static RuaPerDevFlag attrs_;
       bool& attrs = attrs_.get();
       if (!attrs) {
-        (void)hipFuncSetAttribute(reinterpret_cast<const void*>(&wgrad_imgs<8>), hipFuncAttributeMaxDynamicSharedMemorySize, 160 * 1024);
-        (void)hipFuncSetAttribute(reinterpret_cast<const void*>(&wgrad_imgs<16>), hipFuncAttributeMaxDynamicSharedMemorySize, 160 * 1024);
+        (void)hipFuncSetAttribute(reinterpret_cast<const void*>(&wgrad_imgs<8, false>), hipFuncAttributeMaxDynamicSharedMemorySize, 160 * 1024);
+        (void)hipFuncSetAttribute(reinterpret_cast<const void*>(&wgrad_imgs<16, false>), hipFuncAttributeMaxDynamicSharedMemorySize, 160 * 1024);
+        (void)hipFuncSetAttribute(reinterpret_cast<const void*>(&wgrad_imgs<8, true>), hipFuncAttributeMaxDynamicSharedMemorySize, 160 * 1024);
+        (void)hipFuncSetAttribute(reinterpret_cast<const void*>(&wgrad_imgs<16, true>), hipFuncAttributeMaxDynamicSharedMemorySize, 160 * 1024);
         attrs = true;
       }
-      if (d->W == 8) hipLaunchKernelGGL(wgrad_imgs<8>, dim3((unsigned)(k.nti * k.ntc)), dim3(768), smems_, st_, k);
-      else hipLaunchKernelGGL(wgrad_imgs<16>, dim3((unsigned)(k.nti * k.ntc)), dim3(768), smems_, st_, k);
+      const WgImgK ik{k, d->in_scale, d->in_shift, d->in_relu};
+      const dim3 gs_((unsigned)(k.nti * k.ntc));
+      if (d->in_scale && d->W == 8) hipLaunchKernelGGL((wgrad_imgs<8, true>), gs_, dim3(768), smems_, st_, ik);
+      else if (d->in_scale) hipLaunchKernelGGL((wgrad_imgs<16, true>), gs_, dim3(768), smems_, st_, ik);
+      else if (d->W == 8) hipLaunchKernelGGL((wgrad_imgs<8, false>), gs_, dim3(768), smems_, st_, ik);
+      else hipLaunchKernelGGL((wgrad_imgs<16, false>), gs_, dim3(768), smems_, st_, ik);
       RUA_LAUNCH_CHECK("wgrad_imgs");
       return RUA_OK;
     }
@@ -1912,16 +1970,21 @@
     if (k.slabs) note_pending(2, k.ksplit, ndw_, k.slabs, d->dw, 0, (int)((ndw_ / 4 + SLAB_RED_COLS - 1) / SLAB_RED_COLS));
     if (g_wgrad_dry) return RUA_OK;
     const unsigned grid_ = (unsigned)(k.ntc * k.nti * k.ksplit);
-    constexpr int smem_ = 2 * 512 * 128 + 2 * 18 * 128;
+    constexpr int smem_ = 2 * 512 * 128 + 2 * 18 * 128, smem_bn_ = smem_ + 512;
     static RuaPerDevFlag attr_;
     bool& attr = attr_.get();
     if (!attr) {
-      (void)hipFuncSetAttribute(reinterpret_cast<const void*>(&wgrad_img<8>), hipFuncAttributeMaxDynamicSharedMemorySize, 160 * 1024);
-      (void)hipFuncSetAttribute(reinterpret_cast<const void*>(&wgrad_img<16>), hipFuncAttributeMaxDynamicSharedMemorySize, 160 * 1024);
+      (void)hipFuncSetAttribute(reinterpret_cast<const void*>(&wgrad_img<8, false>), hipFuncAttributeMaxDynamicSharedMemorySize, 160 * 1024);
+      (void)hipFuncSetAttribute(reinterpret_cast<const void*>(&wgrad_img<16, false>), hipFuncAttributeMaxDynamicSharedMemorySize, 160 * 1024);
+      (void)hipFuncSetAttribute(reinterpret_cast<const void*>(&wgrad_img<8, true>), hipFuncAttributeMaxDynamicSharedMemorySize, 160 * 1024);
+      (void)hipFuncSetAttribute(reinterpret_cast<const void*>(&wgrad_img<16, true>), hipFuncAttributeMaxDynamicSharedMemorySize, 160 * 1024);
       attr = true;
     }
-    if (d->W == 8) hipLaunchKernelGGL(wgrad_img<8>, dim3(grid_), dim3(768), smem_, st_, k);
-    else hipLaunchKernelGGL(wgrad_img<16>, dim3(grid_), dim3(768), smem_, st_, k);
+    const WgImgK ik{k, d->in_scale, d->in_shift, d->in_relu};
+    if (d->in_scale && d->W == 8) hipLaunchKernelGGL((wgrad_img<8, true>), dim3(grid_), dim3(768), smem_bn_, st_, ik);
+    else if (d->in_scale) hipLaunchKernelGGL((wgrad_img<16, true>), dim3(grid_), dim3(768), smem_bn_, st_, ik);
+    else if (d->W == 8) hipLaunchKernelGGL((wgrad_img<8, false>), dim3(grid_), dim3(768), smem_, st_, ik);
+    else hipLaunchKernelGGL((wgrad_img<16, false>), dim3(grid_), dim3(768), smem_, st_, ik);
     RUA_LAUNCH_CHECK("wgrad_img");
     if (k.slabs && !d->defer) { rua_record_mid_event(st_); return launch_slab_reduce(k.slabs, d->dw, ndw_, k.ksplit, st_); }
     return RUA_OK;
diff --git a/resunet_a_mltsk_keras_amd/engine.py b/resunet_a_mltsk_keras_amd/engine.py
--- a/resunet_a_mltsk_keras_amd/engine.py
+++ b/resunet_a_mltsk_keras_amd/engine.py
@@ -546,13 +546,14 @@
         sg.x, sg.w, sg.C, sg.Hs, sg.Ws, sg.up_shift, sg.dil, sg.taps = x.ptr, x.ptr, x.C, x.H, x.W, 0, dil, 9
         d.N, d.H, d.W, d.Cout, d.stride, d.dtype = x.N, x.H, x.W, nf, 1, self.dt
         d.y, d.out_stride, d.OH, d.OW = x.ptr, 1, x.H, x.W
+        self._ws(d)
         w = L.WgradDesc()
         w.a, w.C, w.Hs, w.Ws, w.dy, w.Cout, w.H, w.W = x.ptr, x.C, x.H, x.W, x.ptr, nf, x.H, x.W
         w.N, w.stride, w.dil, w.taps, w.dtype = x.N, 1, dil, 9, self.dt
         sc = self.e.scratch
         w.workspace, w.workspace_bytes = sc.data_ptr(), sc.numel() * 4
         lib = L.lib()
-        return lib.raw("rua_conv_fused_input_ok")(C.byref(d)) == 1 and lib.raw("rua_wgrad_kind")(C.byref(w)) == 1
+        return lib.raw("rua_conv_fused_input_ok")(C.byref(d)) == 1 and lib.raw("rua_wgrad_fused_input_ok")(C.byref(w)) == 1
 
     def _ws(self, d):
         if not self.dry and self.e.split_k and d.N * d.H * d.W * d.Cout * 4 <= self.e.workspace.numel() * 4:
```

Result: no change. 1330 patches/s (-0.4%).
